# DaehwanKimLab/hisat2

Hardware: AMD Instinct MI355X
Metric: reads/sec, 101 bp PE, REDUCED-SIZE (256000000 bp, GRCh38 contig profile) linear index, --no-spliced-alignment: HI_Aligner::go per pair on the GPU (inputs and report events resident in HBM), SAM-identical to hisat2 (higher is better)
Workload: dtype u32

## Files before the change

hisat2_amd/api.py:

```python
from __future__ import annotations

import ctypes as C
import os

import numpy as np

_HERE = os.path.dirname(os.path.abspath(__file__))
DEFAULT_TAIL, DEFAULT_ALIGN_MATE = 16, 0
LIB_PATH = os.environ.get("H2G_LIBPATH") or os.path.join(_HERE, "libh2g.so")
MAX = 0xFFFFFFFF
MAX_EDITS = 32
SEED_CAP = 5

u32, u8, i32, u64, i64 = C.c_uint32, C.c_uint8, C.c_int32, C.c_uint64, C.c_int64


class LoadOpts(C.Structure):
    _fields_ = [("device", i32), ("load_local", i32)]


class IndexInfo(C.Structure):
    _fields_ = [("len", u32), ("gbwtLen", u32), ("numNodes", u32), ("lineRate", i32), ("offRate", i32),
                ("ftabChars", i32), ("eftabLen", u32), ("linear", u32), ("sideSz", u32), ("sideGbwtSz", u32),
                ("sideGbwtLen", u32), ("numSides", u32), ("offsLen", u32), ("ftabLen", u32), ("nPat", u32),
# ... 416 lines not shown
    L.h2g_rank_bench_synth.argtypes = [vp, C.c_size_t, u64, C.c_int, C.c_int, P(C.c_float), P(u64)]
    L.h2g_rank_bench_synth_sample.argtypes = [vp, C.c_size_t, C.c_size_t, vp]
    L.h2g_fm_search.argtypes = [vp, vp, C.c_size_t, u32, vp]
    L.h2g_sa_resolve.argtypes = [vp, vp, C.c_size_t, u32, vp, vp]
    L.h2g_sw_align.argtypes = [vp, vp, C.c_size_t, vp, C.c_int, P(C.c_float)]
    L.h2g_adjust_with_alt.argtypes = [vp, vp, C.c_size_t, u32, vp, vp]
    L.h2g_sa_resolve_graph.argtypes = [vp, vp, vp, C.c_size_t, u32, vp, vp]
    L.h2g_graph_lf.argtypes = [vp, vp, C.c_size_t, u32, vp, vp]
    L.h2g_fm_search_graph.argtypes = [vp, vp, C.c_size_t, u32, u32, vp, vp]
    L.h2g_index_synth_graph_sides.argtypes = [u64, u64, C.c_int, P(vp)]
    L.h2g_extend.argtypes = [vp, vp, vp, C.c_size_t, vp]
    L.h2g_seed_params_init.argtypes = [P(SeedParams), vp, C.c_int]
    L.h2g_seed_params_init.restype = None
    L.h2g_seed_extend_run.argtypes = [vp, P(SeedParams)]
    L.h2g_seed_extend_fetch.argtypes = [vp, vp, C.c_size_t, C.c_size_t]
    L.h2g_get_counters.argtypes = [vp, P(Counters)]
    L.h2g_align_params_init.argtypes = [P(AlignParams), vp]
    L.h2g_align_params_init.restype = None
    L.h2g_align_option_arity.argtypes = [C.c_char_p]
    L.h2g_align_params_apply_options.argtypes = [P(AlignParams), P(AlignPresets), P(C.c_char_p), C.c_size_t, C.c_char_p, C.c_size_t]
    L.h2g_align_params_presets.argtypes = [P(AlignParams), C.c_int, P(AlignPresets)]
    L.h2g_align_params_presets.restype = None
    L.h2g_ext_search.argtypes = [vp, vp, C.c_size_t, u32, vp, vp]
    L.h2g_local_index_of.argtypes = [vp, u32, u32]
    L.h2g_local_index_of.restype = u32
    L.h2g_set_read_names.argtypes = [vp, C.c_char_p, vp, C.c_size_t]
    L.h2g_align_run.argtypes = [vp, P(AlignParams)]
    L.h2g_align_fetch.argtypes = [vp, vp, vp, C.c_size_t, C.c_size_t]
    L.h2g_set_mates.argtypes = [vp, vp, vp, vp, C.c_char_p, vp, C.c_size_t]
    L.h2g_set_read_seeds.argtypes = [vp, vp, vp, C.c_size_t]
    L.h2g_set_read_filter.argtypes = [vp, vp, vp]
    L.h2g_set_read_ids.argtypes = [vp, vp]
    L.h2g_window_plan_create.argtypes = [u32, u32, u64, P(vp)]
    L.h2g_window_plan_add_file.argtypes = [vp, C.c_char_p, C.c_size_t]
    L.h2g_window_plan_get_info.argtypes = [vp, P(WindowPlanInfo)]
    L.h2g_window_plan_text.argtypes = [vp]
    L.h2g_window_plan_text.restype = vp
    L.h2g_window_plan_prefixes.argtypes = [vp]
    L.h2g_window_plan_prefixes.restype = vp
    L.h2g_window_plan_segments.argtypes = [vp, u64, u64, vp, C.c_size_t]
    L.h2g_window_plan_segments.restype = C.c_size_t
    L.h2g_window_plan_select.argtypes = [vp, u64, u64, P(u64), P(u64)]
    L.h2g_window_plan_select.restype = None
    L.h2g_window_plan_free.argtypes = [vp]
    L.h2g_window_plan_free.restype = None
    L.h2g_set_reads_windows.argtypes = [vp, vp, C.c_size_t, vp, C.c_size_t, u32, u32, vp, C.c_size_t]
    L.h2g_get_windows_stats.argtypes = [vp, P(WindowsStats)]
    L.h2g_fetch_reads.argtypes = [vp, P(C.c_size_t), P(C.c_size_t), P(C.c_size_t), P(C.c_int), vp, vp, vp, vp, vp]
    L.h2g_set_reads_fastq.argtypes = [vp, vp, C.c_size_t, vp, C.c_size_t, P(FastqOpts), P(FastqResult)]
    L.h2g_fetch_read_set.argtypes = [vp, C.c_int, P(C.c_size_t), P(C.c_size_t), P(C.c_size_t), vp, vp, vp, vp, vp]
    L.h2g_get_fastq_stats.argtypes = [vp, P(FastqStats)]
    L.h2g_align_pairs_run.argtypes = [vp, P(AlignParams)]
    sz = C.c_size_t
    L.h2g_sam_plan_unpaired_compact.argtypes = [vp] * 6 + [sz, vp, vp, vp, vp, sz, P(sz), vp, sz, P(sz), vp]
    L.h2g_sam_plan_paired_compact.argtypes = [vp] * 11 + [sz, vp, vp, vp, vp, vp, u32, vp, sz, P(sz), vp, sz, P(sz), vp]
    L.h2g_sam_text_unpaired.argtypes = [vp, vp, vp, sz, vp, sz, vp, sz, P(sz), vp]
    L.h2g_sam_text_paired.argtypes = [vp, vp, vp, sz, vp, sz, vp, sz, P(sz), vp]
    L.h2g_sam_text_from_plan_host.argtypes = [vp] * 11 + [sz, vp, sz, vp, sz, vp, sz, vp, sz, vp, sz, P(sz), vp]
    L.h2g_get_sam_text_stats.argtypes = [vp, P(SamTextStats)]
    L.h2g_sam_text_unpaired_planned.argtypes = [vp] * 7 + [sz, vp, vp, vp, vp, sz, P(sz), vp, sz, P(sz), vp]
    L.h2g_sam_text_paired_planned.argtypes = [vp] * 12 + [sz, vp, vp, vp, vp, vp, u32, vp, sz, P(sz), vp, sz, P(sz), vp]
    L.h2g_get_sam_plan_stats.argtypes = [vp, P(SamPlanStats), vp, sz]
    L.h2g_sam_plan_split_host.argtypes = [vp] * 11 + [sz, vp, vp, vp, vp, vp, u32, vp, sz, P(sz), vp, sz, P(sz), vp, vp]
    L.h2g_align_pairs_fetch.argtypes = [vp, vp, vp, vp, C.c_size_t, C.c_size_t]
    L.h2g_align_fetch_dense.argtypes = [vp, vp, vp, C.c_size_t, vp, C.c_size_t, C.c_size_t]
    L.h2g_align_pairs_fetch_dense.argtypes = [vp, vp, vp, C.c_size_t, vp, vp, C.c_size_t, vp, C.c_size_t, C.c_size_t]
    _lib = L
    return L


def _chk(rc, what):
    if rc != 0:
        msg = lib().h2g_last_error()
        raise H2GError(f"{what} failed: status {rc} ({msg.decode() if msg else ''})")


def mstreams_policy(units, last_bails, linear, pinned=0, light=2):
    f = lib().h2g_mstreams_policy
    f.argtypes = [C.c_ulonglong, C.c_uint, C.c_int, C.c_uint, C.c_uint]
    f.restype = C.c_uint
    return int(f(int(units), int(last_bails), int(bool(linear)), int(pinned), int(light)))


class WindowPlan:
    def __init__(self, length, step, first_rdid=0):
        self.h = C.c_void_p()
        _chk(lib().h2g_window_plan_create(length, step, first_rdid, C.byref(self.h)), "h2g_window_plan_create")
        self.len, self.step = length, step

    def add_file(self, data: bytes):
        _chk(lib().h2g_window_plan_add_file(self.h, data, len(data)), "h2g_window_plan_add_file")

    def info(self):
        i = WindowPlanInfo()
        _chk(lib().h2g_window_plan_get_info(self.h, C.byref(i)), "h2g_window_plan_get_info")
        return i

    @property
    def n_reads(self):
        return int(self.info().n_reads)

    def text(self):
        n = int(self.info().n_text)
        return np.frombuffer(C.string_at(lib().h2g_window_plan_text(self.h), n), dtype=np.uint8).copy() if n else np.zeros(0, np.uint8)

    def prefixes(self):
        n = int(self.info().n_prefix_bytes)
        return C.string_at(lib().h2g_window_plan_prefixes(self.h), n) if n else b""

    def segments(self, first=0, n=None):
        n = self.n_reads - first if n is None else n
        cnt = lib().h2g_window_plan_segments(self.h, first, n, None, 0)
        out = np.zeros(cnt, dtype=WINDOW_SEG_DTYPE)
        if cnt:
            lib().h2g_window_plan_segments(self.h, first, n, out.ctypes.data, cnt)
        return out

    def select(self, rdid_lo, rdid_hi):
        a, b = C.c_uint64(), C.c_uint64()
        lib().h2g_window_plan_select(self.h, rdid_lo, rdid_hi, C.byref(a), C.byref(b))
        return a.value, b.value

    def close(self):
        if self.h:
            lib().h2g_window_plan_free(self.h)
            self.h = C.c_void_p()


def expand_windows(text, segs, length, step, prefixes):
    text = np.asarray(text, dtype=np.uint8)
    starts, names, ids = [], [], []
    for s in segs:
        j = np.arange(int(s["n_windows"]), dtype=np.uint64)
        starts.append(np.uint64(s["text_start"]) + j * np.uint64(step))
        pre = prefixes[int(s["prefix_start"]):int(s["prefix_start"]) + int(s["prefix_len"])]
        names += [pre + str(int(s["name_off0"]) + int(k) * step).encode() for k in j]
        ids.append(((np.uint64(s["rdid0"]) + j * np.uint64(step)) & np.uint64(0xffffffff)).astype(np.uint32))
    starts = np.concatenate(starts) if starts else np.zeros(0, np.uint64)
    n = len(starts)
    codes = text[(starts[:, None] + np.arange(length, dtype=np.uint64)[None, :]).astype(np.int64)].reshape(-1)
    offs = (np.arange(n + 1, dtype=np.uint64) * np.uint64(length)).astype(np.uint32)
    noffs = np.concatenate([[0], np.cumsum([len(x) for x in names])]).astype(np.uint32)
    return codes, offs, b"".join(names), noffs, (np.concatenate(ids) if ids else np.zeros(0, np.uint32))


class Index:
    def __init__(self, base=None, device=0, synth_sides=None, seed=20260925, graph=False):
        L = lib()
        self.h = C.c_void_p()
        if synth_sides is not None and graph:
            _chk(L.h2g_index_synth_graph_sides(int(synth_sides), int(seed), int(device), C.byref(self.h)),
                 "h2g_index_synth_graph_sides")
        elif synth_sides is not None:
            _chk(L.h2g_index_synth_sides(int(synth_sides), int(seed), int(device), C.byref(self.h)), "h2g_index_synth_sides")
        else:
            o = LoadOpts(device, 1)
            _chk(L.h2g_index_load(base.encode(), C.byref(o), C.byref(self.h)), "h2g_index_load")
        self.info = IndexInfo()
        _chk(L.h2g_index_get_info(self.h, C.byref(self.info)), "h2g_index_get_info")

    def dense_sa(self, verify=False):
        st, nd = u32(0), u64(0)
        _chk(lib().h2g_index_dense_sa_check(self.h, C.byref(st), C.byref(nd) if verify else None), "h2g_index_dense_sa_check")
        return bool(st.value), (int(nd.value) if verify else None)

    def dense_lsa(self, verify=False):
# ... 452 lines not shown
```

hisat2_amd/csrc/h2g_go_args.h:

```cpp
#pragma once
#include <hip/hip_runtime.h>
#include <atomic>
#include "h2g_align.h"
#include "h2g_graph.h"
#include "h2g_fast.h"

enum : unsigned {
	H2G_CNT_RANK = 0, H2G_CNT_SIDE = 1, H2G_CNT_STEPS = 2, H2G_CNT_EXT = 3,
	H2G_CNT_ALIGNED = 4, H2G_CNT_OVERFLOW = 5,
	H2G_CNT_FAST_DONE = 6, H2G_CNT_FAST_BAILED = 7,
	H2G_CNT_BENCH_SUM = 6, H2G_CNT_BENCH_CHECKSUM = 7,
	H2G_CNT_WORK_FAST = 12, H2G_CNT_WORK_DRAIN = 13, H2G_CNT_WORK_MAIN = 14, H2G_CNT_WORK_SECOND = 15,
	H2G_CNT_PROF_GO = 16, H2G_CNT_PROF_GO_CTL = 80,
	H2G_CNT_NO_SECOND = 64,
	H2G_CNT_FAST_BAIL_WHY = 96,
	H2G_CNT_FAST_RANK = 120, H2G_CNT_FAST_SIDE = 121, H2G_CNT_FAST_STEPS = 122, H2G_CNT_FAST_ALIGNED = 123,
	H2G_CNT_DRAIN_OFF = 120,
	H2G_CNT_OVF_CURSOR = 124, H2G_CNT_LEDITS_CURSOR = 126,
	H2G_CNT_PROF_FAST = 128, H2G_CNT_PROF_FAST_SITE = 176, H2G_CNT_PROF_FAST_TRIPS = 208,
	H2G_CNT_SECOND = 256,
	H2G_CNT_PROF_FAST_BINS = 512,
#ifdef H2G_GO_PROF
	H2G_CNT_BLOCK = 1024
#else
// ... 70 lines not shown
			uint16_t v;
			while((v = __atomic_load_n(&ring[q][pos], __ATOMIC_RELAXED)) == EMPTY) __builtin_amdgcn_s_sleep(1);
			__atomic_store_n(&ring[q][pos], EMPTY, __ATOMIC_RELAXED);
			*slot = v;
		}
		return n;
	}
};

template <auto K, class... Args>
static int launch_large_lds(unsigned grid, unsigned threads, unsigned lds, hipStream_t st, const Args&... args) {
	static std::atomic<unsigned long long> lds_ok{0};
	int dev = 0; (void)hipGetDevice(&dev);
	const unsigned long long bit = 1ull << (dev & 63);
	if(!(lds_ok.load(std::memory_order_relaxed) & bit)) { if(hipFuncSetAttribute((const void*)K, hipFuncAttributeMaxDynamicSharedMemorySize, 160 * 1024) != hipSuccess) (void)hipGetLastError(); lds_ok.fetch_or(bit, std::memory_order_relaxed); }
	hipLaunchKernelGGL(K, dim3(grid), dim3(threads), lds, st, args...);
	return (int)hipGetLastError();
}

struct GoArgs {
	h2g::DGfm g; h2g::DRef ref; h2g::DLocalSet ls; h2g::DAlts alts; h2g::DSpliceDB ssdb;
	h2g::DReads rd1, rd2;
	h2g::AlnParams P;
	const char* names1; const uint32_t* noffs1;
	const char* names2; const uint32_t* noffs2;
	uint8_t* pool; size_t ws_stride;
	size_t slot_off, gsl_off;
	uint8_t* gws_base; size_t gws_stride;
	uint8_t* sw_base; size_t sw_stride;
	uint8_t* sc_base;
	h2g::MachOut O;
	unsigned long long* counters;
	uint32_t* work;
	const uint32_t* list;
	const uint32_t* nlist;
	uint32_t paired;
	uint32_t dbg_read; uint32_t* dbg_buf;
	uint32_t rdid_base;
	uint32_t defer_overflow;
};
#define H2G_PK_LANE_WORDS_HOST (H2G_PK_WORDS + H2G_PK_WORDS / 2)

struct GoUnitDesc {
	size_t ws_bytes, slot_off, gsl_off;
	size_t gws_bytes;
	int waves;
	uint32_t threads, slots;
	uint32_t lds_ring_bytes, lds_pack_bytes;
	uint32_t caps[5];
	size_t (*sw_bytes)(uint32_t maxlen, int wide);
	int (*launch)(const GoArgs*, const h2g::DExonTbl*, const h2g::XlPairs*, unsigned grid, hipStream_t);
};
#define H2G_GO_DECLARE(NAME) extern "C" const GoUnitDesc* h2g_go_unit_##NAME();
H2G_GO_DECLARE(linear) H2G_GO_DECLARE(graph) H2G_GO_DECLARE(linear_big) H2G_GO_DECLARE(graph_big)
H2G_GO_DECLARE(linear_spl) H2G_GO_DECLARE(linear_spl_big) H2G_GO_DECLARE(graph_spl) H2G_GO_DECLARE(graph_spl_big)
H2G_GO_DECLARE(linear_xl) H2G_GO_DECLARE(graph_xl) H2G_GO_DECLARE(linear_spl_xl) H2G_GO_DECLARE(graph_spl_xl)

struct FastArgs {
	h2g::DGfm g; h2g::DRef ref; h2g::DLocalSet ls;
	h2g::DReads rd1, rd2;
	h2g::AlnParams P;
	const char* names1; const uint32_t* noffs1;
	const char* names2; const uint32_t* noffs2;
	uint32_t* slots;
	h2g::FastOut O;
	unsigned long long* counters;
	uint32_t* work;
	uint32_t* bail_list; uint32_t* bail_count;
	uint32_t total, paired;
	h2g::DAlts alts;
	uint8_t* gws_base; size_t gws_stride;
	uint8_t* sc_base;
	uint32_t tail;
	uint32_t dbg_read; uint32_t* dbg_buf;
	uint32_t orphan_T; uint32_t* orphan_list; uint32_t* orphan_count;
	const uint32_t* adopt_list; const uint32_t* adopt_count; const uint32_t* adopt_slots;
	uint32_t cnt_off;
	uint32_t adopt_slot_words;
	uint32_t mate_handover;
	h2g::DSpliceDB ssdb;
	uint32_t rdid_base;
	uint32_t* ps0;
};
extern "C" int h2g_ps0_launch(const FastArgs* a, uint32_t units, bool paired, hipStream_t st);
struct FastUnitDesc {
	int (*launch)(const FastArgs* a, unsigned grid, hipStream_t);
	int (*launch_drain)(const FastArgs* a, unsigned grid, hipStream_t);
	uint32_t threads, lds_bytes;
	uint32_t slots, slot_bytes;
	uint32_t gws_bytes;
};
extern "C" const FastUnitDesc* h2g_go_fast_unit();
extern "C" const FastUnitDesc* h2g_go_fast_am_unit();
extern "C" const FastUnitDesc* h2g_go_fast_graph_unit();
extern "C" const FastUnitDesc* h2g_go_fast_spl_unit();
```

hisat2_amd/csrc/h2g_k_ps0.hip:

```cpp
#include "h2g_go_args.h"

using namespace h2g;

#define PS0_THREADS 256

__global__ __launch_bounds__(PS0_THREADS, 6) void k_ps0(const FastArgs* __restrict__ A, uint32_t units)
{
	__shared__ uint32_t s_pk[H2G_PK_WORDS * PS0_THREADS];
	const bool paired = A->paired != 0;
	const uint32_t sh = paired ? 2u : 1u;
	const uint32_t t = blockIdx.x * PS0_THREADS + threadIdx.x;
	const uint32_t unit = t >> sh, x = t & ((1u << sh) - 1u), mate = x >> 1;
	const uint32_t lane = threadIdx.x & 63u;
	const bool live = unit < units;
	const DReads& rd = mate ? A->rd2 : A->rd1;
	uint32_t* const pk = s_pk + (threadIdx.x & ~1u);
	bool ok = true;
	uint32_t rl = 0;
	if(live) {
		rl = rd.offs[unit + 1] - rd.offs[unit];
		if((x & 1u) == 0) {
			ok = fg_pack_read(rd, unit, pk, PS0_THREADS);
			if(rd.qc && !rd.qc[unit]) ok = false;
		}
	}
	__syncthreads();
	const unsigned long long bad = __ballot(!ok);
	const bool absent = ((bad >> (lane & ~((1u << sh) - 1u))) & ((1ull << (1u << sh)) - 1ull)) != 0;
	if(!live) return;
	uint32_t rec[FG_PS0_WORDS] = {FG_PS0_ABSENT, FG_PS0_ABSENT, FG_PS0_ABSENT, FG_PS0_ABSENT};
	if(!absent) {
		SeqView sv;
		sv.fwc = nullptr; sv.q = nullptr; sv.len = rl; sv.fw = (x & 1u) == 0;
		sv.pk = pk; sv.pk_stride = PS0_THREADS; sv.pk_nomask = true;
		h2g_fm_hit fh;
		partial_search_item(A->g, sv, 0, A->P.pseudogeneStop != 0, A->P.anchorStop != 0, A->P.khits, &fh);
		fg_ps0_pack(fh, rec);
	}
	*reinterpret_cast<uint4*>(A->ps0 + ((size_t)unit * 4 + x) * FG_PS0_WORDS) = make_uint4(rec[0], rec[1], rec[2], rec[3]);
}

extern "C" int h2g_ps0_launch(const FastArgs* a, uint32_t units, bool paired, hipStream_t st) {
	if(units == 0) return 0;
	const unsigned long long lanes = (unsigned long long)units * (paired ? 4u : 2u);
	hipLaunchKernelGGL(k_ps0, dim3((unsigned)((lanes + PS0_THREADS - 1) / PS0_THREADS)), dim3(PS0_THREADS), 0, st, a, units);
	return (int)hipGetLastError();
}
```

hisat2_amd/csrc/h2g_kernels.hip:

```cpp
#include <hip/hip_runtime.h>
#include <stdio.h>
#include <stdlib.h>
#include <string>
#include <vector>
#include <thread>
#include <atomic>
#include <memory>
#include <chrono>
#include <algorithm>
#define H2G_EXT_OPTS 0
#define H2G_HAPLOTYPE 0
#include "h2g_core.h"
#include "h2g_dev.h"
#include "h2g_parts.h"
#include "h2g_host_index.h"
#include "h2g_align.h"
#include "h2g_graph.h"
#include "h2g_sw.h"
#include "h2g_graph_staged.h"
#include "h2g_local_pack.h"
#include "h2g_splice_host.h"
#include "h2g_splice_db_host.h"
#include "h2g_windows.h"
#include "h2g_fastq.h"
// ... 2 lines not shown
#include <chrono>
#include "h2g_go_args.h"

using namespace h2g;

static thread_local char g_err[512] = "";
static int set_err(const char* what, hipError_t e) {
	snprintf(g_err, sizeof g_err, "%s: %s", what, hipGetErrorString(e));
	return H2G_ERR_DEVICE;
}
#define HIPCHK(call) do { hipError_t e_ = (call); if(e_ != hipSuccess) return set_err(#call, e_); } while(0)

extern "C" const char* h2g_last_error(void) { return g_err; }

struct h2g_index {
	DevStream dense_st;
	HostIndex host;
	bool synthetic = false;
	int device = 0;
	DGfm dg;
	DRef dr;
	DLocalSet dls;
	DAlts dalts;
	bool has_local = false;
	uint32_t n_local = 0;
	bool has_splice_alts = false;
	std::vector<h2g_splice_site> alt_sites;
	DSpliceDB dssdb;
	DExonTbl dexons;
	DevBuf<uint8_t> d_ssdb[4];
	HostSpliceDB h_ssdb;
	const float* d_spl[3] = {nullptr, nullptr, nullptr};
	std::vector<DLocalDesc> h_ldesc;
	std::vector<DevBuf<uint8_t>> allocs;
	uint64_t device_bytes = 0;
	uint32_t* d_sa_dense = nullptr; uint8_t* d_sa_dist = nullptr;
	DevEvent dense_ev;
	std::atomic<bool> dense_ready{false};
	double dense_ms = 0.0;
	bool dense_synced = false;
	uint32_t* d_lsa = nullptr; uint64_t* d_lsa_base = nullptr;
	uint64_t lsa_rows = 0;
	DevEvent lsa_ev;
	std::atomic<bool> lsa_ready{false};
	double lsa_ms = 0.0;
	~h2g_index() { if(dense_st) { (void)hipSetDevice(device); (void)hipStreamSynchronize(dense_st); } }
};
struct IndexFree { void operator()(h2g_index* ix) const { h2g_index_free(ix); } };
typedef std::unique_ptr<h2g_index, IndexFree> IndexPtr;
static DGfm dg_now(h2g_index* ix) {
	DGfm g = ix->dg;
	if(!ix->d_sa_dist) return g;
	if(!ix->dense_ready.load(std::memory_order_acquire)) {
		if(hipEventQuery(ix->dense_ev) != hipSuccess) { (void)hipGetLastError(); return g; }
		ix->dense_ready.store(true, std::memory_order_release);
	}
	g.sa_dense = ix->d_sa_dense; g.sa_dist = ix->d_sa_dist;
	return g;
}

static DLocalSet dls_now(h2g_index* ix) {
	DLocalSet l = ix->dls;
	if(!ix->d_lsa) return l;
	if(!ix->lsa_ready.load(std::memory_order_acquire)) {
		if(hipEventQuery(ix->lsa_ev) != hipSuccess) { (void)hipGetLastError(); return l; }
		ix->lsa_ready.store(true, std::memory_order_release);
	}
	l.lsa = ix->d_lsa; l.lsa_base = ix->d_lsa_base;
	return l;
}

#define H2G_MSTREAMS_MAX 8
#define H2G_MSTREAMS_LIGHT_DEFAULT 2
#define H2G_NBUF (H2G_MSTREAMS_MAX + 1)
#define H2G_FAST_RESERVE_DEFAULT 0
#define H2G_DEFAULT_TAIL 16
#define H2G_ORPHAN_T 512
#define H2G_ORPHAN_MIN_UNITS 200000
#define H2G_DRAIN_GRID 64
#define H2G_FAST_POOLS 3
#ifndef H2G_DEFAULT_PS0
#define H2G_DEFAULT_PS0 1
#endif
#define H2G_DEFAULT_ALIGN_MATE 0
#define H2G_DEFAULT_FAST_SPLICED 0
#define H2G_MACH_MAXGRID 48u
#define H2G_MACH_TOTAL 128u
#define H2G_MAX_BATCHES 16
struct BatchCtx {
	size_t n_reads = 0; uint32_t max_read_len = 0;
	DevBuf<uint8_t> d_codes; DevBuf<uint32_t> d_offs; DevBuf<char> d_quals; bool has_quals = false;
	DevBuf<char> d_names; DevBuf<uint32_t> d_name_offs; bool has_names = false;
	DevBuf<uint8_t> d_codes2; DevBuf<uint32_t> d_offs2; DevBuf<char> d_quals2, d_names2; DevBuf<uint32_t> d_name_offs2; bool has_mates = false, has_quals2 = false;
	DevBuf<ReadOut> d_rout; DevBuf<h2g_alnres> d_aln; uint32_t aln_slots = 0;
	DevBuf<PairOut> d_pout; DevBuf<h2g_alnres> d_paln[2]; uint32_t pair_slots = 0;
	DevBuf<uint32_t> d_seeds; bool has_seeds = false, has_seeds2 = false;
	DevBuf<uint8_t> d_qc; bool has_qc = false;
	DevBuf<uint32_t> d_ids; bool has_ids = false;
	hipError_t ensure_reads(size_t max_reads, size_t max_bases) {
		hipError_t e = d_codes.ensure(max_bases + 64);
		if(e == hipSuccess) e = d_quals.ensure(max_bases + 64);
		return e != hipSuccess ? e : d_offs.ensure(max_reads + 1);
	}
	hipError_t reserve_names(size_t nb, size_t max_reads) {
		if(d_names.size() >= nb + 64 && d_name_offs) return hipSuccess;
		const hipError_t e = d_names.reset(nb + 64);
		return e != hipSuccess ? e : d_name_offs.reset(max_reads + 1);
	}
	hipError_t ensure_mates(size_t max_reads, size_t max_bases, size_t nb2) {
		hipError_t e = d_codes2.ensure(max_bases + 64);
		if(e == hipSuccess) e = d_quals2.ensure(max_bases + 64);
		if(e == hipSuccess) e = d_offs2.ensure(max_reads + 1);
		if(e == hipSuccess) e = d_name_offs2.ensure(max_reads + 1);
		return e != hipSuccess ? e : d_names2.reset(nb2 + 64);
	}
};
enum Tm {
	TM_PRIM0, TM_PRIM1,
	TM_SEED0, TM_SEED_MID, TM_SEED1,
	TM_RUN0, TM_MAIN1, TM_MAIN0, TM_RUN1,
	TM_EXT1,
	TM_FAST1,
	TM_SET0, TM_SET1,
	TM_N
};
struct h2g_stream {
	h2g_index* ix = nullptr;
	DevStream st;
	DevStream mst[H2G_MSTREAMS_MAX];
	DevStream dst;
	unsigned n_mst = 0;
	unsigned mstreams = 0;
	unsigned mstreams_light = H2G_MSTREAMS_LIGHT_DEFAULT;
	unsigned rot = 0;
	bool st2_busy = false;
	unsigned gen = 0;
	struct RunSet {
		DevEvent ev_fast, ev_mach;
		DevEvent ev_bails;
		DevEvent ev_drain;
		DevBuf<uint32_t> bail_list;
		DevBuf<uint32_t> orphans;
		DevBuf<FastArgs> fast_args, drain_args;
	} run[H2G_NBUF];
	DevBuf<unsigned long long> d_counters;
	PinnedBuf<uint32_t> h_bails;
	PinnedBuf<FastArgs> h_fast_args;
	unsigned long long* counters(const RunSet& b) const { return d_counters + (&b - run) * H2G_CNT_BLOCK; }
	uint32_t& h_bail(const RunSet& b) const { return h_bails[&b - run]; }
	FastArgs* h_fast(const RunSet& b) const { return h_fast_args + 2 * (&b - run); }
	FastArgs* h_drain(const RunSet& b) const { return h_fast_args + 2 * (&b - run) + 1; }
	unsigned long long* cnt_cur = nullptr;
	uint32_t last_bails = 0;
	size_t max_reads = 0, max_bases = 0;
	BatchCtx batch[H2G_MAX_BATCHES];
	unsigned cur_batch = 0;
	BatchCtx& cur() { return batch[cur_batch]; }
	const BatchCtx& cur() const { return batch[cur_batch]; }
	DevBuf<h2g_seed_result> d_seed;
	struct GoPool {
		DevBuf<uint8_t> ws;
		DevBuf<uint8_t> gws;
		DevBuf<uint8_t> sw; size_t sw_stride = 0, sw_lanes = 0;
		DevBuf<uint8_t> sc;
	};
	struct MachStream {
		DevEvent ev_rot;
		GoPool main, second;
		DevBuf<uint32_t> ovf_list;
		bool warmed = false;
	} mach[H2G_MSTREAMS_MAX];
	hipStream_t stream_of(const MachStream& m) const { return mst[&m - mach]; }
	const MachStream* ovf_cur = mach;
	DevBuf<uint32_t> dbg_buf;
	struct FastPool {
		DevBuf<uint8_t> slots;
		DevBuf<uint32_t> ps0;
		DevEvent ev_last;
	} fpool[H2G_FAST_POOLS];
	size_t orphan_cap = 0;
	DevBuf<uint8_t> d_drain_slots;
	DevBuf<uint8_t> d_drain_sc;
	bool dst_busy = false;
	DevEvent ev_dr[2];
	bool ran_drain = false;
	const uint32_t* orph_cur = nullptr;
	DevBuf<uint8_t> d_fast_gws;
	DevBuf<uint8_t> d_fast_sc;
	bool ran_fast = false;
	struct Tune { int fast, blocks_per_cu, pair_slots, no_second_pass; unsigned mach_div, mach_min, mach_total; int mach_total_auto = 1; int fast_reserve; long dbg_read;
	              int tail, tail_auto = 1, align_mate, orphan, drain_grid, mate_handover, ps0, fast_spliced; } tune = {};
	h2g_align_params last_p; int last_paired = -1;
	DevBuf<uint8_t> d_sw_ws;
	DevBuf<SwLaneState> d_sw_states;
	PartArea<h2g_edit> ledits; DevBuf<uint32_t> d_ledits_cur;
	unsigned ledits_touched = 0;
	PartArea<h2g_alnres> paln_ovf;
	DevBuf<uint32_t> d_xlp_at; PartArea<uint32_t> xlp; DevBuf<uint32_t> d_xlp_cur;
	const PairOut* xlp_pout = nullptr;
	DevBuf<uint8_t> d_tmp[4];
	uint64_t tmp_gen = 0;
	struct CompactFetch { bool valid = false, paired = false; uint64_t gen = 0; unsigned batch = 0; size_t first = 0, n = 0; const uint8_t* d_rec[2] = {nullptr, nullptr}; uint64_t bytes[2] = {0, 0};
	                      const uint64_t* d_boffs[2] = {nullptr, nullptr};  } cfetch;
	DevBuf<uint8_t> d_sam[5];
	uint64_t samtab_uid = 0, samtab_gen = 0; uint32_t samtab_nrefs = 0, samtab_names = 0, samtab_rg = 0, samtab_nalts = 0; int32_t samtab_strand = 0;
	DevEvent ev_sam[4];
	h2g_sam_text_stats sam_stats = {};
	DevBuf<uint8_t> d_plan[5];
	DevEvent ev_plan[4];
	h2g_sam_plan_stats plan_stats = {};
	std::vector<uint8_t> plan_classes;
	DevEvent tm[TM_N];
	bool ran_seed = false, ran_align = false;
	h2g_counters last;
	h2g_windows_stats win_stats = {};
	h2g_fastq_stats fq_stats = {};
	DevBuf<unsigned long long> d_warm_cnt;
	DevBuf<uint8_t> d_warm_rows;
	~h2g_stream() {
		if(st) (void)hipStreamSynchronize(st);
		if(dst) (void)hipStreamSynchronize(dst);
		for(unsigned k = 0; k < n_mst; k++) (void)hipStreamSynchronize(mst[k]);
	}
};
struct StreamFree { void operator()(h2g_stream* s) const { h2g_stream_free(s); } };

struct Stager {
	enum { T = 6, NB = 2 };
	static constexpr size_t CH = (size_t)16 << 20;
	DevStream st[T]; PinnedBuf<uint8_t> buf[T][NB]; DevEvent ev[T][NB];
	int device = 0; bool ok = false;
	bool init(int dev) {
		device = dev; ok = true;
		for(int t = 0; t < T && ok; t++) {
			ok = st[t].create(hipStreamNonBlocking) == hipSuccess;
			for(int b = 0; b < NB && ok; b++) ok = buf[t][b].ensure(CH) == hipSuccess && ev[t][b].create(hipEventDisableTiming) == hipSuccess;
		}
		if(!ok) (void)hipGetLastError();
		return ok;
	}
	bool copy(void* dst, const void* src, size_t bytes) {
		return gather(dst, bytes, [src](uint8_t* out, size_t off, size_t len) { memcpy(out, (const uint8_t*)src + off, len); });
	}
	template <class F>
	bool gather(void* dst, size_t bytes, F fill) {
		std::atomic<bool> good{true};
		std::thread th[T];
		const size_t nch = (bytes + CH - 1) / CH;
		for(int t = 0; t < T; t++) th[t] = std::thread([&, t]() {
			if(hipSetDevice(device) != hipSuccess) { good = false; return; }
			size_t n = 0;
			for(size_t k = (size_t)t; k < nch; k += T, n++) {
				const int b = (int)(n % NB);
				const size_t off = k * CH, len = bytes - off < CH ? bytes - off : CH;
				if(n >= NB && hipEventSynchronize(ev[t][b]) != hipSuccess) { good = false; return; }
				fill(buf[t][b], off, len);
				if(hipMemcpyAsync((uint8_t*)dst + off, buf[t][b], len, hipMemcpyHostToDevice, st[t]) != hipSuccess || hipEventRecord(ev[t][b], st[t]) != hipSuccess) { good = false; return; }
			}
			if(hipStreamSynchronize(st[t]) != hipSuccess) good = false;
		});
		for(int t = 0; t < T; t++) th[t].join();
		if(!good) (void)hipGetLastError();
		return good;
	}
};
static int index_alloc(h2g_index* ix, size_t bytes, uint8_t** out) {
	DevBuf<uint8_t> b;
	HIPCHK(b.reset(bytes));
	*out = b;
	ix->allocs.push_back(std::move(b));
	ix->device_bytes += bytes;
	return H2G_OK;
}
static int upload_raw(h2g_index* ix, const void* src, size_t n, const void** out, size_t pad, Stager* sg) {
	uint8_t* p = nullptr;
	int rc;
	if((rc = index_alloc(ix, n + pad, &p))) return rc;
	HIPCHK(hipMemset(p + n, 0, pad));
	if(n) {
		if(sg && sg->ok && n >= ((size_t)32 << 20)) { if(!sg->copy(p, src, n)) { snprintf(g_err, sizeof g_err, "index upload through the staging buffers failed"); return H2G_ERR_DEVICE; } }
		else HIPCHK(hipMemcpy(p, src, n, hipMemcpyHostToDevice));
	}
	*out = p;
	return H2G_OK;
}
template <typename T>
static int upload(h2g_index* ix, const std::vector<T>& v, const T** out, size_t pad = 64, Stager* sg = nullptr) {
	const void* p = nullptr;
	const int rc = upload_raw(ix, v.data(), v.size() * sizeof(T), &p, pad ? pad : 64, sg);
	*out = (const T*)p;
	return rc;
}

extern "C" void h2g_load_opts_init(h2g_load_opts* o) { o->device = 0; o->load_local = 1; }

#define H2G_DENSE_CHUNK 4096u
__global__ __launch_bounds__(256) void k_sa_dense_build(DGfm g, uint32_t* sa_dense, uint8_t* sa_dist) {
	const uint64_t wave = (blockIdx.x * (uint64_t)blockDim.x + threadIdx.x) / 64u;
	const uint64_t base = wave * H2G_DENSE_CHUNK;
	if(base >= g.gbwtLen) return;
	const uint64_t lim = base + H2G_DENSE_CHUNK < g.gbwtLen ? base + H2G_DENSE_CHUNK : g.gbwtLen;
	sa_dense_build_rows(g, base + (threadIdx.x & 63u), 64u, lim, sa_dense, sa_dist);
}
__global__ __launch_bounds__(256) void k_sa_dense_check(DGfm g, const uint32_t* sa_dense, const uint8_t* sa_dist, unsigned long long* ndiff) {
	const uint64_t stride = (uint64_t)gridDim.x * blockDim.x;
// ... 406 lines not shown
__global__ void k_synth_write(uint8_t* sides, const uint32_t* cnt, uint64_t nsides, const uint32_t* chunk, uint32_t sideSz) {
	uint64_t t = blockIdx.x * (uint64_t)blockDim.x + threadIdx.x;
	if(t >= SYNTH_CHUNKS) return;
	uint64_t per = (nsides + SYNTH_CHUNKS - 1) / SYNTH_CHUNKS, a = t * per, b = a + per < nsides ? a + per : nsides;
	uint32_t run[4];
	for(int k = 0; k < 4; k++) run[k] = chunk[t * 4 + k];
	for(uint64_t s = a; s < b; s++) {
		uint32_t* occ = reinterpret_cast<uint32_t*>(sides + s * sideSz + sideSz - 16);
		for(int k = 0; k < 4; k++) { occ[k] = run[k]; run[k] += cnt[s * 4 + k]; }
	}
}

static h2g_status synth_sides(uint64_t num_sides, uint64_t seed, int device, uint32_t sideSz, h2g_index** out) {
	const uint32_t syms = sideSz == 64 ? 192u : H2G_GSIDE_SYMS;
	if(!out || num_sides == 0 || num_sides * (uint64_t)syms >= 0xffffffffull) return H2G_ERR_ARG;
	int ndev = 0;
	if(hipGetDeviceCount(&ndev) != hipSuccess || ndev <= 0) { snprintf(g_err, sizeof g_err, "no HIP device"); return H2G_ERR_DEVICE; }
	HIPCHK(hipSetDevice(device));
	IndexPtr ixp(new h2g_index());
	h2g_index* const ix = ixp.get();
	ix->synthetic = true;
	ix->device = device;
	DevBuf<uint8_t> sbuf;
	DevBuf<uint32_t> cnt, tot, chunk;
	const size_t bytes = num_sides * sideSz + 256;
	{
		const char* mt = getenv("H2G_SIDES_MTYPE");
		const bool unc = mt && !strcmp(mt, "uncached");
		if(unc || (mt && !strcmp(mt, "finegrained"))) {
			void* p = nullptr;
			HIPCHK(hipExtMallocWithFlags(&p, bytes, unc ? hipDeviceMallocUncached : hipDeviceMallocFinegrained));
			sbuf = DevBuf<uint8_t>((uint8_t*)p, bytes);
		}
		else HIPCHK(sbuf.reset(bytes));
	}
	uint8_t* const sides = sbuf;
	HIPCHK(cnt.reset(num_sides * 4));
	HIPCHK(tot.reset(4));
	ix->allocs.push_back(std::move(sbuf));
	ix->device_bytes = num_sides * sideSz;
	hipLaunchKernelGGL(k_synth_fill, dim3((unsigned)((num_sides + 255) / 256)), dim3(256), 0, 0, sides, cnt.get(), num_sides, seed, sideSz);
	HIPCHK(chunk.reset(SYNTH_CHUNKS * 4));
	hipLaunchKernelGGL(k_synth_chunk_sum, dim3(SYNTH_CHUNKS / 256), dim3(256), 0, 0, (const uint32_t*)cnt, num_sides, chunk.get());
	hipLaunchKernelGGL(k_synth_chunk_scan, dim3(1), dim3(64), 0, 0, chunk.get(), tot.get());
	hipLaunchKernelGGL(k_synth_write, dim3(SYNTH_CHUNKS / 256), dim3(256), 0, 0, sides, (const uint32_t*)cnt, num_sides, (const uint32_t*)chunk, sideSz);
	uint32_t totals[4];
	HIPCHK(hipMemcpy(totals, tot, 16, hipMemcpyDeviceToHost));
	GfmParams& p = ix->host.g.p;
	uint32_t len = (uint32_t)(num_sides * syms - 1);
	if(sideSz == 64) p.init(len, len + 1, len + 1, 6, 4, 10, 0, 4);
	else p.init(len - 1000, len + 1, len - 500, 7, 4, 10, 0, 4);
	p.numSides = (uint32_t)num_sides;
	ix->host.g.fchr[0] = 0;
	for(int c = 0; c < 4; c++) ix->host.g.fchr[c + 1] = ix->host.g.fchr[c] + totals[c];
	fill_dgfm(ix->host.g, 16, &ix->dg);
	ix->dg.sides = sides;
	ix->dg.nZ = 0;
	*out = ixp.release();
	return H2G_OK;
}
extern "C" h2g_status h2g_index_synth_sides(uint64_t num_sides, uint64_t seed, int device, h2g_index** out) {
	return synth_sides(num_sides, seed, device, 64, out);
}
extern "C" h2g_status h2g_index_synth_graph_sides(uint64_t num_sides, uint64_t seed, int device, h2g_index** out) {
	return synth_sides(num_sides, seed, device, 128, out);
}

struct Knob { const char *key, *env; long def; void (*set)(h2g_stream::Tune&, long); int h2g_stream::Tune::* is_auto; };
#define H2G_KNOB(key, env, def, member, is_auto) {key, env, def, [](h2g_stream::Tune& t, long v) { t.member = (decltype(t.member))v; }, is_auto}
static const Knob g_knobs[] = {
	H2G_KNOB("fast",           "H2G_GO_FAST",            1,                        fast,           nullptr),
	H2G_KNOB("blocks_per_cu",  "H2G_GO_BLOCKS_PER_CU",   0,                        blocks_per_cu,  nullptr),
	H2G_KNOB("pair_slots",     "H2G_PAIR_SLOTS",         0,                        pair_slots,     nullptr),
	H2G_KNOB("no_second_pass", "H2G_GO_NO_SECOND_PASS",  0,                        no_second_pass, nullptr),
	H2G_KNOB("mach_div",       "H2G_MACH_DIV",           0,                        mach_div,       nullptr),
	H2G_KNOB("mach_min",       "H2G_MACH_MIN",           4,                        mach_min,       nullptr),
	H2G_KNOB("dbg_read",       "H2G_GO_DBG_READ",        -1,                       dbg_read,       nullptr),
	H2G_KNOB("tail",           "H2G_FAST_TAIL",          H2G_DEFAULT_TAIL,         tail,           &h2g_stream::Tune::tail_auto),
	H2G_KNOB("align_mate",     "H2G_FAST_AM",            H2G_DEFAULT_ALIGN_MATE,   align_mate,     nullptr),
	H2G_KNOB("orphan",         "H2G_FAST_ORPHAN",        -1,                       orphan,         nullptr),
	H2G_KNOB("drain_grid",     "H2G_DRAIN_GRID",         H2G_DRAIN_GRID,           drain_grid,     nullptr),
	H2G_KNOB("mate_handover",  "H2G_FAST_MATE_HANDOVER", -1,                       mate_handover,  nullptr),
	H2G_KNOB("ps0",            "H2G_FAST_PS0",           -1,                       ps0,            nullptr),
	H2G_KNOB("fast_spliced",   "H2G_FAST_SPLICED",       H2G_DEFAULT_FAST_SPLICED, fast_spliced,   nullptr),
	H2G_KNOB("mach_total",     "H2G_MACH_TOTAL",         H2G_MACH_TOTAL,           mach_total,     &h2g_stream::Tune::mach_total_auto),
	H2G_KNOB("fast_reserve",   "H2G_FAST_RESERVE",       H2G_FAST_RESERVE_DEFAULT, fast_reserve,   nullptr),
};
#undef H2G_KNOB
static unsigned clamp_mstreams(long m) { return (unsigned)(m < 1 ? 1 : m > H2G_MSTREAMS_MAX ? H2G_MSTREAMS_MAX : m); }


extern "C" h2g_status h2g_stream_create(h2g_index* ix, size_t max_reads, size_t max_bases, h2g_stream** out) {
	if(!ix || !out) return H2G_ERR_ARG;
	HIPCHK(hipSetDevice(ix->device));
	std::unique_ptr<h2g_stream, StreamFree> sp(new h2g_stream());
	h2g_stream* const s = sp.get();
	s->ix = ix; s->max_reads = max_reads; s->max_bases = max_bases;
	HIPCHK(s->st.create(hipStreamNonBlocking));
	for(int k = 0; k < H2G_MSTREAMS_MAX; k++) { HIPCHK(s->mst[k].create(hipStreamNonBlocking)); HIPCHK(s->mach[k].ev_rot.create(hipEventDisableTiming)); }
	HIPCHK(s->dst.create(hipStreamNonBlocking));
	HIPCHK(s->h_fast_args.ensure(2 * H2G_NBUF));
	HIPCHK(s->h_bails.ensure(H2G_NBUF)); for(int k = 0; k < H2G_NBUF; k++) s->h_bails[k] = 0;
	for(h2g_stream::RunSet& b : s->run) { HIPCHK(b.ev_fast.create(hipEventDisableTiming)); HIPCHK(b.ev_mach.create(hipEventDisableTiming)); HIPCHK(b.ev_bails.create(hipEventDisableTiming)); HIPCHK(b.ev_drain.create(hipEventDisableTiming)); }
	for(h2g_stream::FastPool& fp : s->fpool) HIPCHK(fp.ev_last.create(hipEventDisableTiming));
	for(int k = 0; k < 2; k++) HIPCHK(s->ev_dr[k].create());
	for(DevEvent& e : s->tm) HIPCHK(e.create());
	HIPCHK(s->d_counters.ensure(H2G_NBUF * H2G_CNT_BLOCK));
	HIPCHK(hipMemset(s->d_counters, 0, s->d_counters.bytes()));
	s->cnt_cur = s->d_counters;
	if(max_reads) {
		HIPCHK(s->batch[0].ensure_reads(max_reads, max_bases));
		HIPCHK(s->d_seed.ensure(max_reads * 2));
		HIPCHK(hipMemset(s->d_seed, 0, s->d_seed.bytes()));
	}
	memset(&s->last, 0, sizeof s->last);
	for(const Knob& k : g_knobs) {
		const char* const e = getenv(k.env);
		k.set(s->tune, e ? atol(e) : k.def);
		if(e && k.is_auto) s->tune.*k.is_auto = 0;
	}
	if(const char* const e = getenv("H2G_MSTREAMS")) s->mstreams = clamp_mstreams(atol(e));
	if(const char* const e = getenv("H2G_MSTREAMS_LIGHT")) s->mstreams_light = clamp_mstreams(atol(e));
	*out = sp.release();
	return H2G_OK;
}

extern "C" void h2g_stream_free(h2g_stream* s) { delete s; }

static hipError_t sync_mach(h2g_stream* s) {
	if(!s->st2_busy) return hipSuccess;
	for(unsigned k = 0; k < s->n_mst; k++) { const hipError_t e = hipStreamSynchronize(s->mst[k]); if(e != hipSuccess) return e; }
	s->st2_busy = false;
	return hipSuccess;
}
static hipError_t sync_all(h2g_stream* s) {
	hipError_t e = hipStreamSynchronize(s->st);
	if(e == hipSuccess && s->dst_busy) { e = hipStreamSynchronize(s->dst); s->dst_busy = false; }
	if(e == hipSuccess && s->st2_busy) { e = sync_mach(s); s->st2_busy = false; }
	return e;
}
extern "C" void* h2g_stream_hip(h2g_stream* s) { return s ? (void*)s->st : nullptr; }
extern "C" h2g_status h2g_stream_sync(h2g_stream* s) {
	if(!s) return H2G_ERR_ARG;
	HIPCHK(sync_all(s));
	return H2G_OK;
}

extern "C" h2g_status h2g_stream_select_batch(h2g_stream* s, unsigned k) {
	if(!s || k >= H2G_MAX_BATCHES) return H2G_ERR_ARG;
	if(k == s->cur_batch) return H2G_OK;
	HIPCHK(hipSetDevice(s->ix->device));
	const BatchCtx& out = s->cur();
	BatchCtx& in = s->batch[k];
	if(s->max_reads) HIPCHK(in.ensure_reads(s->max_reads, s->max_bases));
	if(!in.d_paln[1] && out.d_pout && out.d_paln[1]) {
		HIPCHK(in.d_pout.ensure(s->max_reads));
		for(int m = 0; m < 2; m++) HIPCHK(in.d_paln[m].reserve(out.d_paln[m].size()));
		in.pair_slots = out.pair_slots;
		HIPCHK(hipMemsetAsync(in.d_pout, 0, in.d_pout.bytes(), s->st));
		for(int m = 0; m < 2; m++) HIPCHK(hipMemsetAsync(in.d_paln[m], 0, in.d_paln[m].bytes(), s->st));
	}
	if(!in.d_aln && out.d_rout && out.d_aln) {
		HIPCHK(in.d_rout.ensure(s->max_reads));
		HIPCHK(in.d_aln.reserve(out.d_aln.size()));
		in.aln_slots = out.aln_slots;
		HIPCHK(hipMemsetAsync(in.d_rout, 0, in.d_rout.bytes(), s->st));
		HIPCHK(hipMemsetAsync(in.d_aln, 0, in.d_aln.bytes(), s->st));
	}
	s->cur_batch = k;
	s->tmp_gen++;
	return H2G_OK;
}

static int tmp_buf(h2g_stream* s, int slot, size_t bytes, void** out) {
	s->tmp_gen++;
	const hipError_t e = s->d_tmp[slot].reserve(bytes + 256);
	*out = s->d_tmp[slot];
	return e == hipSuccess ? H2G_OK : set_err("tmp_buf", e);
}

extern "C" h2g_status h2g_set_reads(h2g_stream* s, const uint8_t* codes, const uint32_t* offs, const char* quals, size_t n) {
	if(s) HIPCHK(sync_all(s));
	if(!s || !codes || !offs || n > s->max_reads) return H2G_ERR_ARG;
	s->tmp_gen++;
	BatchCtx& B = s->cur();
	size_t nb = offs[n];
	if(nb > s->max_bases) return H2G_ERR_ARG;
	uint32_t mx = 0;
	for(size_t i = 0; i < n; i++) { const uint32_t l = offs[i + 1] - offs[i]; if(l > mx) mx = l; }
	B.max_read_len = mx;
	HIPCHK(hipMemcpyAsync(B.d_codes, codes, nb, hipMemcpyHostToDevice, s->st));
	HIPCHK(hipMemcpyAsync(B.d_offs, offs, (n + 1) * 4, hipMemcpyHostToDevice, s->st));
	B.has_quals = quals != nullptr;
	if(quals) HIPCHK(hipMemcpyAsync(B.d_quals, quals, nb, hipMemcpyHostToDevice, s->st));
	HIPCHK(sync_all(s));
	B.n_reads = n;
	B.has_names = false;
	B.has_mates = false;
	B.has_seeds = B.has_seeds2 = false;
	B.has_qc = false;
	B.has_ids = false;
	s->ledits_touched = 0;
	return H2G_OK;
}

static DReads dreads(const h2g_stream* s) {
	DReads r;
	r.codes = s->cur().d_codes; r.offs = s->cur().d_offs; r.quals = s->cur().has_quals ? s->cur().d_quals : nullptr; r.n = (uint32_t)s->cur().n_reads;
	return r;
}

static unsigned grid_for(size_t n, unsigned block) {
	size_t g = (n + block - 1) / block;
	const size_t cap = 256 * 16;
	return (unsigned)(g < 1 ? 1 : (g > cap ? cap : g));
}

__device__ __forceinline__ uint32_t synth_row(uint64_t h, uint32_t n) { return (uint32_t)(((h >> 32) * (uint64_t)n) >> 32); }
__global__ __launch_bounds__(256) void k_rank_v0(DGfm g, const uint32_t* rows, const uint8_t* cs, uint32_t* out,
                                                 size_t n, uint64_t seed, int synth)
{
	size_t stride = (size_t)gridDim.x * blockDim.x;
	for(size_t i = blockIdx.x * (size_t)blockDim.x + threadIdx.x; i < n; i += stride) {
		uint32_t row; int c;
		if(synth) { uint64_t h = splitmix64(seed + i); row = synth_row(h, g.gbwtLen); c = (int)((h >> 40) & 3); }
		else { row = rows[i]; c = cs[i]; }
		out[i] = rank64(g, row, c);
	}
}

__global__ __launch_bounds__(512) void k_rank_v0_512(DGfm g, const uint32_t* rows, const uint8_t* cs, uint32_t* out, size_t n, uint64_t seed, int synth)
{
	size_t stride = (size_t)gridDim.x * blockDim.x;
	for(size_t i = blockIdx.x * (size_t)blockDim.x + threadIdx.x; i < n; i += stride) {
		uint32_t row; int c;
		if(synth) { uint64_t h = splitmix64(seed + i); row = synth_row(h, g.gbwtLen); c = (int)((h >> 40) & 3); }
		else { row = rows[i]; c = cs[i]; }
		out[i] = rank64(g, row, c);
	}
}

__global__ __launch_bounds__(256) void k_rank_v0_sampled(DGfm g, uint32_t* out, size_t n, uint64_t seed, unsigned long long* sum)
{
	size_t stride = (size_t)gridDim.x * blockDim.x;
	unsigned long long acc = 0;
	for(size_t i = blockIdx.x * (size_t)blockDim.x + threadIdx.x; i < n; i += stride) {
		const uint64_t h = splitmix64(seed + i);
		const uint32_t r = rank64(g, synth_row(h, g.gbwtLen), (int)((h >> 40) & 3));
		if((i & 255) == 0) out[i] = r;
		acc += (unsigned long long)r * (unsigned long long)((i & 1023) + 1);
	}
	for(int o = 32; o > 0; o >>= 1) acc += __shfl_xor(acc, o);
	if((threadIdx.x & 63) == 0) atomicAdd(sum, acc);
}

template <int UNROLL>
__global__ __launch_bounds__(256) void k_rank_v1(DGfm g, const uint32_t* rows, const uint8_t* cs, uint32_t* out,
                                                 size_t n, uint64_t seed, int synth)
{
	const unsigned lane = threadIdx.x & 63, sub = lane & 3;
	const size_t ngroups = ((size_t)gridDim.x * blockDim.x) >> 2;
	const size_t gid = (blockIdx.x * (size_t)blockDim.x + threadIdx.x) >> 2;
	for(size_t base = gid * UNROLL; base < n; base += ngroups * UNROLL) {
		uint32_t row[UNROLL], sideNum[UNROLL], charOff[UNROLL]; int c[UNROLL]; uint4 v[UNROLL];
#pragma unroll
		for(int u = 0; u < UNROLL; u++) {
			size_t i = base + u;
			bool ok = i < n;
			if(synth) { uint64_t h = splitmix64(seed + (ok ? i : 0)); row[u] = synth_row(h, g.gbwtLen); c[u] = (int)((h >> 40) & 3); }
			else { row[u] = ok ? rows[i] : 0; c[u] = ok ? cs[i] : 0; }
			sideNum[u] = row[u] / 192u; charOff[u] = row[u] - sideNum[u] * 192u;
			v[u] = reinterpret_cast<const uint4*>(g.sides + (size_t)sideNum[u] * 64)[sub];
		}
#pragma unroll
		for(int u = 0; u < UNROLL; u++) {
			uint64_t w0 = v[u].x | ((uint64_t)v[u].y << 32), w1 = v[u].z | ((uint64_t)v[u].w << 32);
			int n0 = (int)charOff[u] - 64 * (int)sub;
// ... 953 lines not shown
	h2g_ghit scratch;
	for(size_t i = blockIdx.x * (size_t)blockDim.x + threadIdx.x; i < n; i += stride) {
		SeqView sv = seq_view(rd, (uint32_t)(i >> 1), (i & 1) == 0);
		resolve_extend_item(g, ref, sc, sv, &out[i], &scratch);
		nsteps += out[i].nsteps; next += out[i].ncoords;
	}
	wave_add(counters + H2G_CNT_STEPS, nsteps);
	wave_add(counters + H2G_CNT_EXT, next);
}

extern "C" void h2g_seed_params_init(h2g_seed_params* p, const h2g_index* ix, int no_spliced) {
	p->pseudogeneStop = (ix && ix->dg.linear && !no_spliced) ? 1 : 0;
	p->anchorStop = 1;
	p->khits = (ix && !ix->dg.linear) ? 10 : 5;
	p->search_variant = 0;
}

extern "C" h2g_status h2g_seed_extend_run(h2g_stream* s, const h2g_seed_params* p) {
	if(!s || !p) return H2G_ERR_ARG;
	int rc;
	if((rc = need_reads(s)) || (rc = need_linear(s))) return rc;
	HIPCHK(hipSetDevice(s->ix->device));
	const size_t n = s->cur().n_reads * 2;
	HIPCHK(hipMemsetAsync(s->d_counters, 0, 4 * sizeof(unsigned long long), s->st));
	DScoring sc;
	HIPCHK(hipEventRecord(s->tm[TM_SEED0], s->st));
	hipLaunchKernelGGL(k_seed_search, dim3(grid_for(n, 256)), dim3(256), 0, s->st, s->ix->dg, dreads(s), *p, s->d_seed, s->d_counters);
	HIPCHK(hipEventRecord(s->tm[TM_SEED_MID], s->st));
	hipLaunchKernelGGL(k_seed_resolve_extend, dim3(grid_for(n, 256)), dim3(256), 0, s->st, dg_now(s->ix), s->ix->dr, dreads(s), sc, s->d_seed, s->d_counters);
	HIPCHK(hipEventRecord(s->tm[TM_SEED1], s->st));
	HIPCHK(hipGetLastError());
	s->ran_seed = true;
	return H2G_OK;
}

extern "C" h2g_status h2g_seed_extend_fetch(h2g_stream* s, h2g_seed_result* out, size_t first_read, size_t n_reads) {
	if(!s || !out || first_read + n_reads > s->cur().n_reads) return H2G_ERR_ARG;
	HIPCHK(hipMemcpyAsync(out, s->d_seed + first_read * 2, n_reads * 2 * sizeof *out, hipMemcpyDeviceToHost, s->st));
	HIPCHK(sync_all(s));
	return H2G_OK;
}

static_assert(sizeof(h2g_alnres) == sizeof(AlnRec), "h2g_alnres must mirror AlnRec");
static_assert(sizeof(h2g_read_result) == 40, "h2g_read_result layout");
static_assert(sizeof(h2g_pair_result) == sizeof(PairOut), "h2g_pair_result must mirror PairOut");
static_assert(H2G_PAIR_CAP == AL_MAX_PAIRS, "pair capacity");

extern "C" int h2g_device_count(void) { int n = 0; if(hipGetDeviceCount(&n) != hipSuccess) { (void)hipGetLastError(); return 0; } return n; }

extern "C" void h2g_align_params_init(h2g_align_params* p, const h2g_index* ix) { align_params_defaults(p, !ix || ix->dg.linear); }

extern "C" h2g_status h2g_set_read_names(h2g_stream* s, const char* bytes, const uint32_t* offs, size_t n) {
	if(s) HIPCHK(sync_all(s));
	if(!s || !bytes || !offs || n != s->cur().n_reads || n == 0) return H2G_ERR_ARG;
	s->tmp_gen++;
	HIPCHK(hipSetDevice(s->ix->device));
	BatchCtx& B = s->cur();
	size_t nb = offs[n];
	HIPCHK(B.reserve_names(nb, s->max_reads));
	HIPCHK(hipMemcpyAsync(B.d_names, bytes, nb, hipMemcpyHostToDevice, s->st));
	HIPCHK(hipMemcpyAsync(B.d_name_offs, offs, (n + 1) * 4, hipMemcpyHostToDevice, s->st));
	HIPCHK(sync_all(s));
	B.has_names = true;
	return H2G_OK;
}

extern "C" h2g_status h2g_set_mates(h2g_stream* s, const uint8_t* codes2, const uint32_t* offs2, const char* quals2,
                                    const char* nb2, const uint32_t* noffs2, size_t n)
{
	if(s) HIPCHK(sync_all(s));
	if(!s || !codes2 || !offs2 || !nb2 || !noffs2 || n != s->cur().n_reads || n == 0) return H2G_ERR_ARG;
	if(offs2[n] > s->max_bases) return H2G_ERR_ARG;
	s->tmp_gen++;
	BatchCtx& B = s->cur();
	for(size_t i = 0; i < n; i++) { const uint32_t l = offs2[i + 1] - offs2[i]; if(l > B.max_read_len) B.max_read_len = l; }
	HIPCHK(hipSetDevice(s->ix->device));
	HIPCHK(B.ensure_mates(s->max_reads, s->max_bases, noffs2[n]));
	HIPCHK(hipMemcpyAsync(B.d_codes2, codes2, offs2[n], hipMemcpyHostToDevice, s->st));
	HIPCHK(hipMemcpyAsync(B.d_offs2, offs2, (n + 1) * 4, hipMemcpyHostToDevice, s->st));
	B.has_quals2 = quals2 != nullptr;
	if(quals2) HIPCHK(hipMemcpyAsync(B.d_quals2, quals2, offs2[n], hipMemcpyHostToDevice, s->st));
	HIPCHK(hipMemcpyAsync(B.d_names2, nb2, noffs2[n], hipMemcpyHostToDevice, s->st));
	HIPCHK(hipMemcpyAsync(B.d_name_offs2, noffs2, (n + 1) * 4, hipMemcpyHostToDevice, s->st));
	HIPCHK(sync_all(s));
	B.has_mates = true;
	return H2G_OK;
}

extern "C" h2g_status h2g_set_read_seeds(h2g_stream* s, const uint32_t* seeds1, const uint32_t* seeds2, size_t n) {
	if(s) HIPCHK(sync_all(s));
	if(!s) return H2G_ERR_ARG;
	BatchCtx& B = s->cur();
	if(!seeds1) { B.has_seeds = B.has_seeds2 = false; return H2G_OK; }
	if(n != B.n_reads || n == 0) return H2G_ERR_ARG;
	HIPCHK(hipSetDevice(s->ix->device));
	HIPCHK(B.d_seeds.ensure(2 * s->max_reads));
	HIPCHK(hipMemcpyAsync(B.d_seeds, seeds1, n * sizeof(uint32_t), hipMemcpyHostToDevice, s->st));
	if(seeds2) HIPCHK(hipMemcpyAsync(B.d_seeds + s->max_reads, seeds2, n * sizeof(uint32_t), hipMemcpyHostToDevice, s->st));
	HIPCHK(sync_all(s));
	B.has_seeds = true; B.has_seeds2 = seeds2 != nullptr;
	return H2G_OK;
}

extern "C" h2g_status h2g_set_read_ids(h2g_stream* s, const uint32_t* ids) {
	if(s) HIPCHK(sync_all(s));
	if(!s) return H2G_ERR_ARG;
	BatchCtx& B = s->cur();
	if(!ids) { B.has_ids = false; return H2G_OK; }
	const size_t n = B.n_reads;
	if(n == 0 || n > s->max_reads) return H2G_ERR_ARG;
	HIPCHK(hipSetDevice(s->ix->device));
	HIPCHK(B.d_ids.ensure(s->max_reads));
	HIPCHK(hipMemcpyAsync(B.d_ids, ids, n * sizeof(uint32_t), hipMemcpyHostToDevice, s->st));
	HIPCHK(sync_all(s));
	B.has_ids = true;
	return H2G_OK;
}

__global__ __launch_bounds__(256) void k_win_codes(const uint8_t* __restrict__ text, const h2g_win::DSeg* __restrict__ segs, uint32_t n_segs, uint32_t len, uint32_t step,
                                                   uint64_t n_bytes, uint8_t* __restrict__ codes)
{
	const uint64_t chunks = (n_bytes + 15) / 16;
	for(uint64_t c = (uint64_t)blockIdx.x * blockDim.x + threadIdx.x; c < chunks; c += (uint64_t)gridDim.x * blockDim.x) {
		const uint64_t b0 = c * 16;
		const uint32_t m = n_bytes - b0 < 16 ? (uint32_t)(n_bytes - b0) : 16u;
		h2g_win::CodeCursor cur;
		cur.seek(segs, n_segs, len, step, b0);
		uint32_t w[4] = {0, 0, 0, 0};
		for(uint32_t k = 0; k < m; k++) w[k >> 2] |= (uint32_t)text[cur.next()] << (8 * (k & 3));
		*(uint4*)(codes + b0) = make_uint4(w[0], w[1], w[2], w[3]);
	}
}
__global__ __launch_bounds__(256) void k_win_meta(const h2g_win::DSeg* __restrict__ segs, uint32_t n_segs, uint32_t len, uint32_t step, uint32_t n, const char* __restrict__ prefixes,
                                                  uint32_t* __restrict__ offs, uint32_t* __restrict__ ids, uint32_t* __restrict__ name_offs, char* __restrict__ names)
{
	for(uint32_t r = blockIdx.x * blockDim.x + threadIdx.x; r <= n; r += gridDim.x * blockDim.x) {
		offs[r] = r * len;
		if(r == n) { name_offs[r] = segs[n_segs].name_first; break; }
		const h2g_win::DSeg s = segs[h2g_win::seg_of(segs, n_segs, r)];
		const uint32_t j = r - s.first_read;
		ids[r] = s.rdid0 + j * step;
		const uint32_t at = h2g_win::name_start(s, step, j);
		name_offs[r] = at;
		h2g_win::write_name(s, step, j, prefixes, names + at);
	}
}

extern "C" h2g_status h2g_set_reads_windows(h2g_stream* s, const uint8_t* text, size_t n_text, const h2g_window_seg* segs, size_t n_segs, uint32_t len, uint32_t step,
                                            const char* prefixes, size_t n_prefix_bytes)
{
	if(s) HIPCHK(sync_all(s));
	if(!s || !text || !segs || n_segs == 0 || n_segs >= 0xffffffffull || len == 0 || (!prefixes && n_prefix_bytes)) return H2G_ERR_ARG;
	s->tmp_gen++;
	BatchCtx& B = s->cur();
	std::vector<h2g_win::DSeg> ds(n_segs + 1);
	uint64_t n = 0, nb = 0, lo = UINT64_MAX, hi = 0;
	for(size_t k = 0; k < n_segs; k++) {
		const h2g_window_seg& x = segs[k];
		const uint64_t last = x.text_start + (uint64_t)(x.n_windows ? x.n_windows - 1 : 0) * step;
		if(x.n_windows == 0 || last + len > n_text || last < x.text_start || (uint64_t)x.prefix_start + x.prefix_len > n_prefix_bytes) {
			snprintf(g_err, sizeof g_err, "h2g_set_reads_windows: segment %zu names text or prefix bytes that were not given", k); return H2G_ERR_ARG;
		}
		if(x.text_start < lo) lo = x.text_start;
		if(last + len > hi) hi = last + len;
		h2g_win::DSeg& d = ds[k];
		d.name_off0 = x.name_off0; d.rdid0 = (uint32_t)x.rdid0; d.first_read = (uint32_t)n; d.name_first = (uint32_t)nb;
		d.prefix_start = x.prefix_start; d.prefix_len = x.prefix_len;
		n += x.n_windows;
		nb += (uint64_t)x.n_windows * x.prefix_len + h2g_win::width_sum(x.name_off0, step, x.n_windows);
		if(n > s->max_reads || n * len > s->max_bases || n * len > 0xffffffffull || nb > 0xffffffffull) {
			snprintf(g_err, sizeof g_err, "h2g_set_reads_windows: the windows exceed the stream's %zu reads / %zu bases, or their names 4 GB", s->max_reads, s->max_bases); return H2G_ERR_ARG;
		}
	}
	if(hi - lo > 0xffffffffull) { snprintf(g_err, sizeof g_err, "h2g_set_reads_windows: the segments span more than 4 G bases of text"); return H2G_ERR_ARG; }
	for(size_t k = 0; k < n_segs; k++) ds[k].text_start = (uint32_t)(segs[k].text_start - lo);
	memset(&ds[n_segs], 0, sizeof ds[n_segs]);
	ds[n_segs].first_read = (uint32_t)n; ds[n_segs].name_first = (uint32_t)nb;
	HIPCHK(hipSetDevice(s->ix->device));
	HIPCHK(B.reserve_names(nb, s->max_reads));
	HIPCHK(B.d_ids.ensure(s->max_reads));
	void *d_text, *d_segs, *d_pre;
	int rc;
	if((rc = tmp_buf(s, 0, hi - lo, &d_text)) || (rc = tmp_buf(s, 1, ds.size() * sizeof(h2g_win::DSeg), &d_segs)) || (rc = tmp_buf(s, 2, n_prefix_bytes, &d_pre))) return (h2g_status)rc;
	HIPCHK(hipMemcpyAsync(d_text, text + lo, hi - lo, hipMemcpyHostToDevice, s->st));
	HIPCHK(hipMemcpyAsync(d_segs, ds.data(), ds.size() * sizeof(h2g_win::DSeg), hipMemcpyHostToDevice, s->st));
	if(n_prefix_bytes) HIPCHK(hipMemcpyAsync(d_pre, prefixes, n_prefix_bytes, hipMemcpyHostToDevice, s->st));
	const uint64_t n_bytes = n * len;
	HIPCHK(hipEventRecord(s->tm[TM_SET0], s->st));
	k_win_codes<<<grid_for((n_bytes + 15) / 16, 256), 256, 0, s->st>>>((const uint8_t*)d_text, (const h2g_win::DSeg*)d_segs, (uint32_t)n_segs, len, step, n_bytes, B.d_codes);
	k_win_meta<<<grid_for(n + 1, 256), 256, 0, s->st>>>((const h2g_win::DSeg*)d_segs, (uint32_t)n_segs, len, step, (uint32_t)n, (const char*)d_pre, B.d_offs, B.d_ids, B.d_name_offs, B.d_names);
	HIPCHK(hipGetLastError());
	HIPCHK(hipEventRecord(s->tm[TM_SET1], s->st));
	HIPCHK(sync_all(s));
	s->win_stats.bytes_uploaded = (hi - lo) + ds.size() * sizeof(h2g_win::DSeg) + n_prefix_bytes;
	s->win_stats.bytes_written = n_bytes + (n + 1) * 8 + n * 4 + nb;
	HIPCHK(hipEventElapsedTime(&s->win_stats.kernel_ms, s->tm[TM_SET0], s->tm[TM_SET1]));
	B.n_reads = n;
	B.max_read_len = len;
	B.has_quals = false;
	B.has_names = true;
	B.has_mates = false;
	B.has_seeds = B.has_seeds2 = false;
	B.has_qc = false;
	B.has_ids = true;
	s->ledits_touched = 0;
	return H2G_OK;
}
extern "C" h2g_status h2g_get_windows_stats(h2g_stream* s, h2g_windows_stats* out) {
	if(!s || !out) return H2G_ERR_ARG;
	*out = s->win_stats;
	return H2G_OK;
}

extern "C" h2g_status h2g_fetch_reads(h2g_stream* s, size_t* n_reads, size_t* n_bases, size_t* n_name_bytes, int* has_ids, uint8_t* codes, uint32_t* offs, char* names,
                                      uint32_t* name_offs, uint32_t* ids)
{
	if(!s) return H2G_ERR_ARG;
	HIPCHK(sync_all(s));
	const BatchCtx& B = s->cur();
	const size_t n = B.n_reads;
	uint32_t nb = 0, nn = 0;
	HIPCHK(hipSetDevice(s->ix->device));
	if(n) HIPCHK(hipMemcpy(&nb, B.d_offs + n, 4, hipMemcpyDeviceToHost));
	if(n && B.has_names) HIPCHK(hipMemcpy(&nn, B.d_name_offs + n, 4, hipMemcpyDeviceToHost));
	if(n_reads) *n_reads = n;
	if(n_bases) *n_bases = nb;
	if(n_name_bytes) *n_name_bytes = nn;
	if(has_ids) *has_ids = B.has_ids ? 1 : 0;
	if(n == 0) return H2G_OK;
	if((ids && !B.has_ids) || ((names || name_offs) && !B.has_names)) return H2G_ERR_ARG;
	if(codes && nb) HIPCHK(hipMemcpy(codes, B.d_codes, nb, hipMemcpyDeviceToHost));
	if(offs) HIPCHK(hipMemcpy(offs, B.d_offs, (n + 1) * 4, hipMemcpyDeviceToHost));
	if(names && nn) HIPCHK(hipMemcpy(names, B.d_names, nn, hipMemcpyDeviceToHost));
	if(name_offs) HIPCHK(hipMemcpy(name_offs, B.d_name_offs, (n + 1) * 4, hipMemcpyDeviceToHost));
	if(ids) HIPCHK(hipMemcpy(ids, B.d_ids, n * 4, hipMemcpyDeviceToHost));
	return H2G_OK;
}

extern "C" h2g_status h2g_set_read_filter(h2g_stream* s, const uint8_t* pass1, const uint8_t* pass2) {
	if(s) HIPCHK(sync_all(s));
	if(!s) return H2G_ERR_ARG;
	BatchCtx& B = s->cur();
	if(!pass1 && !pass2) { B.has_qc = false; return H2G_OK; }
	const size_t n = B.n_reads;
	if(n == 0 || n > s->max_reads) return H2G_ERR_ARG;
	HIPCHK(hipSetDevice(s->ix->device));
	HIPCHK(B.d_qc.ensure(2 * s->max_reads));
	if(pass1) HIPCHK(hipMemcpyAsync(B.d_qc, pass1, n, hipMemcpyHostToDevice, s->st)); else HIPCHK(hipMemsetAsync(B.d_qc, 1, n, s->st));
	if(pass2) HIPCHK(hipMemcpyAsync(B.d_qc + s->max_reads, pass2, n, hipMemcpyHostToDevice, s->st)); else HIPCHK(hipMemsetAsync(B.d_qc + s->max_reads, 1, n, s->st));
	HIPCHK(sync_all(s));
	B.has_qc = true;
	return H2G_OK;
}

extern "C" h2g_status h2g_combine_with(h2g_stream* s, const h2g_align_params* p, h2g_ghit* a, const h2g_ghit* b, const int64_t* minsc, size_t n, uint32_t* ok) {
	if(!s || !a || !b || !minsc || !ok || n == 0) return H2G_ERR_ARG;
	int rc;
	if((rc = need_reads(s))) return rc;
	if(s->ix->synthetic) { snprintf(g_err, sizeof g_err, "synthetic index: rank only"); return H2G_ERR_ARG; }
	const bool linear = s->ix->dg.linear != 0;
	for(size_t i = 0; i < n; i++) {
		if(a[i].read >= s->cur().n_reads || b[i].read != a[i].read || a[i].tidx >= s->ix->dr.nrefs || b[i].tidx >= s->ix->dr.nrefs || a[i].nedits > H2G_MAX_EDITS || b[i].nedits > H2G_MAX_EDITS) return H2G_ERR_ARG;
	}
	if(s->cur().max_read_len > H2G_COMBINE_MAXLEN) return H2G_ERR_ARG;
	h2g_align_params hp;
	if(p) hp = *p; else align_params_defaults(&hp, linear);
	AlnParams P = aln_params_from(hp, hp.no_spliced_alignment != 0, linear);
	if(!hp.no_spliced_alignment) { P.sc.donor_sum = s->ix->d_spl[0]; P.sc.acc_sum1 = s->ix->d_spl[1]; P.sc.acc_sum2 = s->ix->d_spl[2]; }
	HIPCHK(hipSetDevice(s->ix->device));
	unsigned grid = grid_for(n, 256);
	if(grid > 64) grid = 64;
	void *da, *db, *dm, *dscr;
	const size_t ab = n * sizeof(h2g_ghit);
	if((rc = tmp_buf(s, 0, 2 * ab, &da)) || (rc = tmp_buf(s, 1, n * 8, &dm)) || (rc = tmp_buf(s, 2, n * 4, &db)) ||
	   (rc = tmp_buf(s, 3, (size_t)grid * 256 * 2 * H2G_COMBINE_MAXLEN * sizeof(int64_t), &dscr))) return rc;
	h2g_ghit* const d_a = (h2g_ghit*)da; h2g_ghit* const d_b = d_a + n;
	HIPCHK(hipMemcpyAsync(d_a, a, ab, hipMemcpyHostToDevice, s->st));
	HIPCHK(hipMemcpyAsync(d_b, b, ab, hipMemcpyHostToDevice, s->st));
	HIPCHK(hipMemcpyAsync(dm, minsc, n * 8, hipMemcpyHostToDevice, s->st));
	hipLaunchKernelGGL(k_combine, dim3(grid), dim3(256), 0, s->st, s->ix->dr, s->ix->dalts, dreads(s), P, d_a, (const h2g_ghit*)d_b, (const int64_t*)dm, n, (uint32_t*)db, (int64_t*)dscr);
	HIPCHK(hipGetLastError());
	HIPCHK(hipMemcpyAsync(a, d_a, ab, hipMemcpyDeviceToHost, s->st));
	HIPCHK(hipMemcpyAsync(ok, db, n * 4, hipMemcpyDeviceToHost, s->st));
	HIPCHK(sync_all(s));
	return H2G_OK;
}

static int need_alignable(h2g_stream* s) {
	if(s->ix->synthetic) { snprintf(g_err, sizeof g_err, "synthetic index: rank only"); return H2G_ERR_ARG; }
	const DGfm& g = s->ix->dg;
	if(g.linear && g.lineRate == 6) return H2G_OK;
	if(!g.linear && g.lineRate == 7) return H2G_OK;
	snprintf(g_err, sizeof g_err, "unsupported side geometry (lineRate %u)", g.lineRate);
	return H2G_ERR_UNSUPPORTED;
}

static const GoUnitDesc& go_unit(bool linear, bool big, bool spliced = false, bool xl = false) {
	static const GoUnitDesc* (*const u[2][2][3])() = {
		{{h2g_go_unit_graph, h2g_go_unit_graph_big, h2g_go_unit_graph_xl}, {h2g_go_unit_linear, h2g_go_unit_linear_big, h2g_go_unit_linear_xl}},
		{{h2g_go_unit_graph_spl, h2g_go_unit_graph_spl_big, h2g_go_unit_graph_spl_xl}, {h2g_go_unit_linear_spl, h2g_go_unit_linear_spl_big, h2g_go_unit_linear_spl_xl}}};
	return *u[spliced ? 1 : 0][linear ? 1 : 0][xl ? 2 : big ? 1 : 0]();
}
static const FastUnitDesc& fast_unit(bool linear, bool spliced, bool align_mate) {
	return *(!linear ? h2g_go_fast_graph_unit : spliced ? h2g_go_fast_spl_unit : align_mate ? h2g_go_fast_am_unit : h2g_go_fast_unit)();
}

static int go_pool_for(h2g_stream* s, h2g_stream::GoPool& pl, const GoUnitDesc& u, size_t slots, size_t lanes, uint32_t bowtie2_dp, GoArgs* a) {
	const size_t wsb = u.ws_bytes, gwb = u.gws_bytes;
	HIPCHK(pl.ws.reserve(slots * wsb));
	a->pool = pl.ws; a->ws_stride = wsb; a->slot_off = u.slot_off; a->gsl_off = u.gsl_off;
	a->gws_base = nullptr; a->gws_stride = gwb;
	if(gwb) {
		HIPCHK(pl.gws.reserve(lanes * gwb));
		a->gws_base = pl.gws;
	}
	HIPCHK(pl.sc.reserve(lanes * (size_t)(2 * H2G_COMBINE_MAXLEN * sizeof(int64_t))));
	a->sc_base = pl.sc;
	a->sw_base = nullptr; a->sw_stride = 0;
	if(bowtie2_dp) {
		const uint32_t swlen = s->cur().max_read_len > H2G_SW_MAX_ROWS ? (uint32_t)H2G_SW_MAX_ROWS : s->cur().max_read_len;
		bool wide = false;
		for(uint32_t l = 1; l <= swlen && !wide; l++) wide = sw_wide_for(min_score_for(a->P, l));
		const size_t stride = (u.sw_bytes(swlen, wide ? 1 : 0) + 255) & ~(size_t)255;
		if(pl.sw_stride < stride || pl.sw_lanes < lanes) {
			pl.sw_stride = 0; pl.sw_lanes = 0;
			HIPCHK(pl.sw.reset(stride * lanes));
			HIPCHK(hipMemset(pl.sw, 0, stride * lanes));
			pl.sw_stride = stride; pl.sw_lanes = lanes;
		}
		a->sw_base = pl.sw; a->sw_stride = pl.sw_stride;
	}
	return H2G_OK;
}


static int go_check(h2g_stream* s, const h2g_align_params* p, bool paired) {
	int rc;
	if((rc = need_reads(s)) || (rc = need_alignable(s))) return rc;
	if(!s->ix->has_local) { snprintf(g_err, sizeof g_err, "align: index loaded without local (.5/.6) indexes"); return H2G_ERR_ARG; }
	if(!s->cur().has_names || (paired && !s->cur().has_mates)) { snprintf(g_err, sizeof g_err, "align: read names (h2g_set_read_names)%s not set", paired ? " / mates (h2g_set_mates)" : ""); return H2G_ERR_ARG; }
	if(paired && s->cur().has_seeds && !s->cur().has_seeds2) { snprintf(g_err, sizeof g_err, "align: explicit seeds without mate 2's (h2g_set_read_seeds seeds2)"); return H2G_ERR_ARG; }
	if(p->n_ceil_type < 1 || p->n_ceil_type > 4) { snprintf(g_err, sizeof g_err, "align: n_ceil_type %u (1 C, 2 L, 3 S, 4 G)", p->n_ceil_type); return H2G_ERR_ARG; }
	if(p->sc_min < 1) { snprintf(g_err, sizeof g_err, "align: sc_min %d (--sp): the soft-clipping penalty must be at least 1", p->sc_min); return H2G_ERR_ARG; }
	if(p->mm_max < 1) { snprintf(g_err, sizeof g_err, "align: mm_max %d (--mp): the maximum mismatch penalty must be at least 1", p->mm_max); return H2G_ERR_ARG; }
	if(p->mm_max < p->mm_min) { snprintf(g_err, sizeof g_err, "align: mm_max %d is less than mm_min %d (--mp)", p->mm_max, p->mm_min); return H2G_ERR_ARG; }
	if(p->rdg_linear < 1 || p->rfg_linear < 1) { snprintf(g_err, sizeof g_err, "align: rdg_linear %d / rfg_linear %d (--rdg, --rfg): a gap extension penalty must be at least 1", p->rdg_linear, p->rfg_linear); return H2G_ERR_ARG; }
	if(!p->no_spliced_alignment) {
		if(p->pen_canintronlen_type < 1 || p->pen_canintronlen_type > 4 || p->pen_noncanintronlen_type < 1 || p->pen_noncanintronlen_type > 4 ||
		   p->min_intronlen < 20 || p->max_intronlen < p->min_intronlen || p->pen_cansplice < 0 || p->pen_noncansplice < 0 ||
		   p->min_anchor_len < 1 || p->min_anchor_len_noncan < 1) {
			snprintf(g_err, sizeof g_err, "align: splice scoring outside its range (intron-length function type 1..4, 20 <= min_intronlen <= max_intronlen, penalties >= 0)");
			return H2G_ERR_ARG;
		}
		if(p->max_intronlen > H2G_SPL_MAXLEN) {
			snprintf(g_err, sizeof g_err, "align: --max-intronlen %u is beyond the %u bases a splice edit holds", p->max_intronlen, (unsigned)H2G_SPL_MAXLEN);
			return H2G_ERR_UNSUPPORTED;
		}
	}
	if(p->khits == 0 || p->khits > H2G_KHITS_MAX || p->kseeds < p->khits || p->kseeds > H2G_KSEEDS_MAX) {
		snprintf(g_err, sizeof g_err, "align: -k %u / --max-seeds %u outside the built range (1 <= -k <= %u, -k <= --max-seeds <= %u)", p->khits, p->kseeds, (unsigned)H2G_KHITS_MAX, (unsigned)H2G_KSEEDS_MAX);
		return H2G_ERR_ARG;
	}
	if(p->bowtie2_dp > 2 || p->pe_orientation > 2 || p->min_frag_len >= (1u << 24)) return H2G_ERR_ARG;
	if(p->pen_conflictsplice < 0) { snprintf(g_err, sizeof g_err, "align: --pen-conflictsplice arg must be at least 0"); return H2G_ERR_ARG; }
	if(p->max_alts_tried && p->max_alts_tried < 8) { snprintf(g_err, sizeof g_err, "align: --max-altstried arg must be at least 8"); return H2G_ERR_ARG; }
	if(p->bowtie2_dp && s->cur().max_read_len == 0) return H2G_ERR_ARG;
	return H2G_OK;
}

struct GoPlan {
	bool linear, spl, xl, big_main, fast, second;
	bool fast_spl;
	const GoUnitDesc *U, *L;
	unsigned grid, M, bgrid;
	unsigned S;
	unsigned mach_cap, pool_cap;
	size_t units;
};
static unsigned mstreams_policy(size_t units, uint32_t last_bails, bool linear, unsigned pinned, unsigned light) {
	if(pinned) return pinned > H2G_MSTREAMS_MAX ? H2G_MSTREAMS_MAX : pinned;
	if(!linear || (size_t)last_bails * 1000 > units * 15) return H2G_MSTREAMS_MAX;
	return light < 1 ? 1u : light > H2G_MSTREAMS_MAX ? (unsigned)H2G_MSTREAMS_MAX : light;
}
extern "C" __attribute__((visibility("default"))) unsigned h2g_mstreams_policy(unsigned long long units, unsigned last_bails, int linear, unsigned pinned, unsigned light) {
	return mstreams_policy((size_t)units, last_bails, linear != 0, pinned, light);
}
static GoPlan go_plan(const h2g_stream* s, const h2g_align_params* p, bool paired) {
	GoPlan plan, *g = &plan;
	const size_t n_reads = s->cur().n_reads;
	g->linear = s->ix->dg.linear != 0;
	const bool ext_opts = pe_flags_from(*p) != H2G_PE_DEFAULT || p->min_frag_len != 0 || p->transcriptome_mapping_only || (p->avoid_pseudogene && !p->no_spliced_alignment);
	g->spl = !p->no_spliced_alignment || (p->use_haplotype && !g->linear) || ext_opts;
	const uint32_t maxsz = p->khits > p->kseeds ? p->khits : p->kseeds;
	g->L = &go_unit(g->linear, true, g->spl);
	const uint32_t* const caps = go_unit(g->linear, false, g->spl).caps, * const bcaps = g->L->caps;
	g->xl = p->khits > H2G_SELECT_CAP || maxsz > bcaps[0];
	g->big_main = maxsz > caps[0];
	g->U = &go_unit(g->linear, g->big_main, g->spl, g->xl);
	g->fast = s->tune.fast && !g->spl && !g->big_main && p->no_spliced_alignment && !p->secondary && !p->bowtie2_dp;
	g->fast_spl = s->tune.fast && s->tune.fast_spliced && g->linear && !p->no_spliced_alignment && !ext_opts && !g->big_main && !p->secondary && !p->bowtie2_dp;
	if(g->fast_spl) g->fast = true;
	g->second = !g->big_main && !s->tune.no_second_pass;
	size_t per_cu = (size_t)g->U->waves * 256 / g->U->threads;
	const size_t lds_blocks = (160u * 1024u) / (g->U->lds_ring_bytes + (paired ? 2u : 1u) * g->U->lds_pack_bytes);
	if(per_cu > lds_blocks) per_cu = lds_blocks;
	if(per_cu < 1) per_cu = 1;
	if(s->tune.blocks_per_cu > 0) per_cu = (size_t)s->tune.blocks_per_cu;
	const size_t want = (n_reads + g->U->slots - 1) / g->U->slots;
	size_t maxblocks = 256 * per_cu;
	if(g->big_main && maxblocks > 32) maxblocks = 32;
	if(g->xl && maxblocks > 12) maxblocks = 12;
	g->grid = (unsigned)(want < 1 ? 1 : (want > maxblocks ? maxblocks : want));
	g->M = s->mstreams ? s->mstreams : H2G_MSTREAMS_MAX;
	const bool mt_auto = s->tune.mach_total_auto != 0 && g->linear;
	g->units = paired ? n_reads : (n_reads + 1) / 2;
	const unsigned mach_total_now = mt_auto && (size_t)s->last_bails * 1000 > g->units * 15 ? 192u : s->tune.mach_total;
	g->S = mstreams_policy(g->units, s->last_bails, g->linear, s->mstreams, s->mstreams_light);
	g->mach_cap = mach_total_now / g->M;
	if(g->mach_cap > H2G_MACH_MAXGRID) g->mach_cap = H2G_MACH_MAXGRID;
	if(g->mach_cap < 1) g->mach_cap = 1;
	g->pool_cap = (mt_auto ? 192u : s->tune.mach_total) / g->M;
	if(g->pool_cap > H2G_MACH_MAXGRID) g->pool_cap = H2G_MACH_MAXGRID;
	if(g->pool_cap < g->mach_cap) g->pool_cap = g->mach_cap;
	g->bgrid = g->fast ? 2u : 4u;
	return plan;
}

struct FastPlan {
	bool use_am, mate_ho;
	bool ps0;
	const FastUnitDesc *FU, *DU;
	unsigned fgrid, mgrid, dgrid;
	uint32_t orphan_T;
	h2g_stream::FastPool* pool;
	size_t slot_bytes;
};
struct GoRun {
	GoArgs A; DExonTbl X; XlPairs XP;
	h2g_stream::RunSet* set;
	unsigned long long* cblk;
	unsigned lane;
	h2g_stream::MachStream* mach;
	hipStream_t ms;
	unsigned mach_grid;
	FastPlan f;
	uint32_t* ovl;
};

static void go_args(const h2g_stream* s, const h2g_align_params* p, bool paired, const GoPlan& g, GoRun* r) {
	const BatchCtx& b = s->cur();
	GoArgs& A = r->A;
	memset(&A, 0, sizeof A);
	A.g = dg_now(s->ix); A.ref = s->ix->dr; A.ls = dls_now(s->ix); A.alts = s->ix->dalts;
	if(p->max_alts_tried) A.alts.maxAltsTried = p->max_alts_tried;
	if(p->use_haplotype && !g.linear && A.alts.n) A.alts.has_splice |= 2u;
	A.rd1 = dreads(s); A.rd2 = A.rd1;
	if(paired) { A.rd2.codes = b.d_codes2; A.rd2.offs = b.d_offs2; A.rd2.quals = b.has_quals2 ? b.d_quals2 : nullptr; }
	if(b.has_seeds) { A.rd1.seeds = b.d_seeds; A.rd2.seeds = paired ? b.d_seeds + s->max_reads : b.d_seeds; }
	if(b.has_ids) { A.rd1.ids = b.d_ids; A.rd2.ids = b.d_ids; }
	if(b.has_qc) { A.rd1.qc = b.d_qc; A.rd2.qc = paired ? b.d_qc + s->max_reads : b.d_qc; }
	A.P = aln_params_from(*p, p->no_spliced_alignment != 0, g.linear);
	if(!p->no_spliced_alignment) { A.ssdb = s->ix->dssdb; A.rdid_base = p->first_read_id; }
	r->X = p->no_spliced_alignment ? DExonTbl() : s->ix->dexons;
	if(!p->no_spliced_alignment) { A.P.sc.donor_sum = s->ix->d_spl[0]; A.P.sc.acc_sum1 = s->ix->d_spl[1]; A.P.sc.acc_sum2 = s->ix->d_spl[2]; }
	A.names1 = b.d_names; A.noffs1 = b.d_name_offs; A.names2 = b.d_names2; A.noffs2 = b.d_name_offs2;
	A.paired = paired ? 1u : 0u;
}

static void go_select(h2g_stream* s, const GoPlan& g, GoRun* r) {
	r->set = &s->run[s->gen % (g.M + 1)];
	r->cblk = s->counters(*r->set);
	r->lane = g.fast ? s->gen % g.M : 0u;
	r->mach = &s->mach[r->lane % g.S];
}

static int go_rotation(h2g_stream* s, const GoPlan& g) {
	if(s->n_mst < g.S) s->n_mst = g.S;
	if(s->rot && s->rot != g.S && s->st2_busy) {
		for(unsigned j = 0; j < s->rot; j++) HIPCHK(hipEventRecord(s->mach[j].ev_rot, s->mst[j]));
		for(unsigned k = 0; k < g.S; k++) for(unsigned j = 0; j < s->rot; j++) if(j != k) HIPCHK(hipStreamWaitEvent(s->mst[k], s->mach[j].ev_rot, 0));
	}
	s->rot = g.S;
	return H2G_OK;
}

static int go_pools(h2g_stream* s, const h2g_align_params* p, const GoPlan& g, GoRun* r) {
	const size_t pgrid = g.fast && g.grid > g.pool_cap ? (size_t)g.pool_cap : (size_t)g.grid;
	int rc;
	if(g.fast && s->cur().n_reads >= 200000) {
		GoArgs scratch = r->A;
		for(unsigned k = 0; k < g.S && s->gen >= 1; k++) {
			h2g_stream::MachStream& m = s->mach[k];
			if((rc = go_pool_for(s, m.main, *g.U, pgrid * g.U->slots, pgrid * g.U->threads, p->bowtie2_dp, &scratch))) return rc;
			if(g.second && (rc = go_pool_for(s, m.second, *g.L, (size_t)g.bgrid * g.L->slots, (size_t)g.bgrid * g.L->threads, p->bowtie2_dp, &scratch))) return rc;
			if(!m.ovf_list) { HIPCHK(m.ovf_list.ensure(s->max_reads + 4)); HIPCHK(hipMemsetAsync(m.ovf_list + s->max_reads, 0, 16, s->stream_of(m))); }
		}
		for(unsigned k = 0; k < g.M + 1; k++) {
			h2g_stream::RunSet& b = s->run[k];
			HIPCHK(b.bail_list.ensure(s->max_reads + 4));
			HIPCHK(b.fast_args.ensure(1));
			HIPCHK(b.drain_args.ensure(1));
		}
	}
	return go_pool_for(s, r->mach->main, *g.U, pgrid * g.U->slots, pgrid * g.U->threads, p->bowtie2_dp, &r->A);
}

static int go_rows(h2g_stream* s, const h2g_align_params* p, bool paired, const GoPlan& g, GoRun* r) {
	BatchCtx& b = s->cur();
	GoArgs& A = r->A;
	memset(&A.O, 0, sizeof A.O);
	if(!paired) {
		HIPCHK(b.d_rout.ensure(s->max_reads));
		const uint32_t slots = p->khits;
		HIPCHK(b.d_aln.reserve(s->max_reads * (size_t)slots));
		b.aln_slots = slots;
		A.O.rout = b.d_rout; A.O.aln = b.d_aln; A.O.aln_slots = slots;
	} else {
		HIPCHK(b.d_pout.ensure(s->max_reads));
		uint32_t pslots = p->khits * 2 + 4;
		if(pslots < H2G_PAIR_RES_CAP) pslots = H2G_PAIR_RES_CAP;
		if(s->tune.pair_slots > 0) pslots = (uint32_t)s->tune.pair_slots;
		for(int m = 0; m < 2; m++) HIPCHK(b.d_paln[m].reserve(s->max_reads * (size_t)pslots));
		b.pair_slots = pslots;
		A.O.pout = b.d_pout; A.O.paln[0] = b.d_paln[0]; A.O.paln[1] = b.d_paln[1]; A.O.pair_slots = pslots;
		const size_t ovf_cap = s->max_reads / 4 > 65536 ? s->max_reads / 4 : 65536;
		if(!s->paln_ovf.fits(g.M, ovf_cap)) {
			HIPCHK(sync_mach(s));
			HIPCHK(hipStreamSynchronize(s->st));
			HIPCHK(s->paln_ovf.reset(g.M, ovf_cap));
		}
		A.O.ovf = s->paln_ovf;
	}
	memset(&r->XP, 0, sizeof r->XP);
	if(paired && g.xl) {
		const size_t xcap = s->max_reads * 64 > ((size_t)1 << 20) ? s->max_reads * 64 : ((size_t)1 << 20);
		if(s->d_xlp_at.size() < s->max_reads || !s->xlp.fits(g.M, xcap) || !s->d_xlp_cur) {
			HIPCHK(hipStreamSynchronize(s->st));
			HIPCHK(s->d_xlp_at.reset(s->max_reads));
			HIPCHK(s->xlp.reset(g.M, xcap));
			HIPCHK(s->d_xlp_cur.ensure(H2G_MSTREAMS_MAX));
		}
		HIPCHK(hipMemsetAsync(s->d_xlp_at, 0, b.n_reads * 4, s->st));
		HIPCHK(hipMemsetD32Async((hipDeviceptr_t)(s->d_xlp_cur + r->lane), (int)s->xlp.lo(r->lane), 1, s->st));
		r->XP.at = s->d_xlp_at; r->XP.list = s->xlp; r->XP.cursor = s->d_xlp_cur + r->lane; r->XP.cap = (uint32_t)s->xlp.hi(r->lane);
	}
	if(paired) s->xlp_pout = g.xl ? b.d_pout : (s->xlp_pout == b.d_pout ? nullptr : s->xlp_pout);
	return H2G_OK;
}

static int go_counters(h2g_stream* s, bool paired, const GoPlan& g, GoRun* r) {
	GoArgs& A = r->A;
	HIPCHK(hipStreamWaitEvent(s->st, r->set->ev_mach, 0));
	HIPCHK(hipMemsetAsync(r->cblk, 0, H2G_CNT_BLOCK * sizeof(unsigned long long), s->st));
	A.counters = r->cblk;
	A.work = reinterpret_cast<uint32_t*>(r->cblk + H2G_CNT_WORK_MAIN);
	if(paired) {
		A.O.ovf_cursor = reinterpret_cast<uint32_t*>(r->cblk + H2G_CNT_OVF_CURSOR);
		A.O.ovf_cap = (uint32_t)s->paln_ovf.hi(r->lane);
		if(r->lane) HIPCHK(hipMemsetD32Async((hipDeviceptr_t)A.O.ovf_cursor, (int)s->paln_ovf.lo(r->lane), 1, s->st));
	}
	A.list = nullptr; A.nlist = nullptr;
	if(s->tune.dbg_read >= 0) {
		HIPCHK(s->dbg_buf.ensure(1u << 20));
		HIPCHK(hipMemsetAsync(s->dbg_buf, 0, (1u << 20) * 4, s->st));
		A.dbg_buf = s->dbg_buf; A.dbg_read = (uint32_t)s->tune.dbg_read;
	}
	A.defer_overflow = g.second ? 1u : 0u;
	return H2G_OK;
}

static void fast_policy(h2g_stream* s, bool paired, const GoPlan& g, FastPlan* f) {
	const size_t n_reads = s->cur().n_reads;
	const bool linear = g.linear;
	*f = FastPlan();
	f->use_am = linear && paired && s->tune.align_mate != 0 && !g.fast_spl;
	f->FU = &fast_unit(linear, g.fast_spl, f->use_am);
	const unsigned NB = g.M + 1;
	for(unsigned back = 1; back < NB && back <= s->gen; back++) {
		const h2g_stream::RunSet& b = s->run[(s->gen - back) % NB];
		if(hipEventQuery(b.ev_bails) == hipSuccess) { s->last_bails = s->h_bail(b); break; }
	}
	(void)hipGetLastError();
	unsigned mach_div = s->tune.mach_div;
	if(mach_div == 0) {
		mach_div = 400;
		if(!linear) {
			const size_t units = paired ? n_reads : n_reads / 2;
			if(units >= 1000000) mach_div = 1600;
			else if(units > 500000) mach_div = 400 + (unsigned)((units - 500000) * 1200 / 500000);
		}
	}
	f->mgrid = (unsigned)((s->last_bails + mach_div - 1) / (mach_div ? mach_div : 1u));
	if(f->mgrid < s->tune.mach_min) f->mgrid = s->tune.mach_min;
	if(f->mgrid > g.mach_cap) f->mgrid = g.mach_cap;
	const size_t fwant = (n_reads + 127) / 128;
	unsigned reserve = s->tune.fast_reserve >= 0 ? (unsigned)s->tune.fast_reserve : g.S * f->mgrid;
	if(reserve > 192) reserve = 192;
	const unsigned fmax = 256 - reserve;
	f->fgrid = (unsigned)(fwant < 1 ? 1 : (fwant > fmax ? fmax : fwant));
	f->slot_bytes = (size_t)256 * f->FU->slots * f->FU->slot_bytes;
	f->orphan_T = s->tune.orphan >= 0 ? (uint32_t)s->tune.orphan : (g.units >= H2G_ORPHAN_MIN_UNITS ? (uint32_t)H2G_ORPHAN_T : 0u);
	if(f->orphan_T > f->FU->slots) f->orphan_T = f->FU->slots;
	if(f->FU->gws_bytes != 0) f->orphan_T = 0;
	f->dgrid = (unsigned)(s->tune.drain_grid < 1 ? 1 : s->tune.drain_grid);
	f->mate_ho = f->orphan_T != 0 && linear && paired && !f->use_am && !g.fast_spl && s->tune.mate_handover != 0;
	f->DU = &fast_unit(linear, g.fast_spl, f->use_am || f->mate_ho);
	f->pool = &s->fpool[f->orphan_T ? s->gen % H2G_FAST_POOLS : 0u];
	f->ps0 = linear && !g.fast_spl && (s->tune.ps0 < 0 ? H2G_DEFAULT_PS0 != 0 : s->tune.ps0 != 0);
}

static int fast_buffers(h2g_stream* s, const GoPlan& g, const FastPlan& f) {
	const size_t ocap = (size_t)256 * f.FU->slots, dbytes = (size_t)f.dgrid * f.DU->slots * f.DU->slot_bytes;
	const size_t dsc = g.linear ? 0 : (size_t)f.dgrid * f.FU->threads * (size_t)(2 * H2G_COMBINE_MAXLEN * sizeof(int64_t));
	h2g_stream::FastPool* const pools = f.orphan_T ? s->fpool : f.pool;
	const unsigned npools = f.orphan_T ? (unsigned)H2G_FAST_POOLS : 1u;
	bool need = f.pool->slots.size() < f.slot_bytes;
	if(f.orphan_T) {
		for(unsigned q = 0; q < npools; q++) need = need || pools[q].slots.size() < f.slot_bytes;
		need = need || s->d_drain_slots.size() < dbytes || s->d_drain_sc.size() < dsc;
		for(unsigned b = 0; b < g.M + 1; b++) need = need || !s->run[b].orphans || !s->run[b].drain_args;
		need = need || s->orphan_cap < ocap;
	}
	const size_t pswords = (size_t)s->max_reads * 4 * FG_PS0_WORDS;
	if(f.ps0) for(unsigned q = 0; q < npools; q++) need = need || pools[q].ps0.size() < pswords;
	if(!need) return H2G_OK;
	HIPCHK(hipStreamSynchronize(s->st)); HIPCHK(hipStreamSynchronize(s->dst)); for(unsigned k = 0; k < s->n_mst; k++) HIPCHK(hipStreamSynchronize(s->mst[k]));
	for(unsigned q = 0; q < npools; q++) {
		DevBuf<uint8_t>& fs = pools[q].slots;
		if(fs.size() < f.slot_bytes) { HIPCHK(fs.reserve(f.slot_bytes)); HIPCHK(hipMemsetAsync(fs, 0, f.slot_bytes, s->st)); }
		DevBuf<uint32_t>& ps = pools[q].ps0;
		if(f.ps0 && ps.size() < pswords) { HIPCHK(ps.reserve(pswords)); HIPCHK(hipMemsetAsync(ps, 0xff, pswords * 4, s->st)); }
	}
	if(f.orphan_T) {
		if(s->orphan_cap < ocap) { for(h2g_stream::RunSet& b : s->run) b.orphans = DevBuf<uint32_t>(); s->orphan_cap = ocap; }
		for(unsigned k = 0; k < g.M + 1; k++) {
			h2g_stream::RunSet& b = s->run[k];
			if(!b.orphans) { HIPCHK(b.orphans.ensure(s->orphan_cap + 4)); HIPCHK(hipMemsetAsync(b.orphans, 0, (s->orphan_cap + 4) * 4, s->st)); }
			HIPCHK(b.drain_args.ensure(1));
		}
		if(s->d_drain_slots.size() < dbytes) { HIPCHK(s->d_drain_slots.reserve(dbytes)); HIPCHK(hipMemsetAsync(s->d_drain_slots, 0, dbytes, s->st)); }
		if(s->d_drain_sc.size() < dsc) { HIPCHK(s->d_drain_sc.reserve(dsc)); HIPCHK(hipMemsetAsync(s->d_drain_sc, 0, dsc, s->st)); }
	}
	HIPCHK(hipStreamSynchronize(s->st));
	return H2G_OK;
}

static int fast_launch(h2g_stream* s, bool paired, const GoPlan& g, GoRun* r) {
	const FastPlan& f = r->f;
	const GoArgs& A = r->A;
	h2g_stream::RunSet& set = *r->set;
	HIPCHK(hipStreamWaitEvent(s->st, f.pool->ev_last, 0));
	HIPCHK(set.bail_list.ensure(s->max_reads + 4));
	uint32_t* const bl = set.bail_list;
	HIPCHK(hipMemsetAsync(bl + s->max_reads, 0, 16, s->st));
	FastArgs F;
	memset(&F, 0, sizeof F);
	F.g = A.g; F.ref = A.ref; F.ls = A.ls; F.rd1 = A.rd1; F.rd2 = A.rd2; F.P = A.P;
	F.names1 = A.names1; F.noffs1 = A.noffs1; F.names2 = A.names2; F.noffs2 = A.noffs2;
	F.slots = (uint32_t*)f.pool->slots.get();
	F.O.rout = A.O.rout; F.O.aln = A.O.aln; F.O.aln_slots = A.O.aln_slots; F.O.pout = A.O.pout; F.O.paln[0] = A.O.paln[0]; F.O.paln[1] = A.O.paln[1]; F.O.pair_slots = A.O.pair_slots;
	F.counters = r->cblk; F.work = reinterpret_cast<uint32_t*>(r->cblk + H2G_CNT_WORK_FAST);
	F.bail_list = bl; F.bail_count = bl + s->max_reads;
	F.total = (uint32_t)s->cur().n_reads; F.paired = paired ? 1u : 0u;
	F.alts = A.alts; F.gws_base = nullptr; F.gws_stride = 0; F.sc_base = nullptr;
	F.dbg_read = A.dbg_read; F.dbg_buf = A.dbg_buf;
	F.ps0 = f.ps0 ? f.pool->ps0.get() : nullptr;
	F.ssdb = A.ssdb; F.rdid_base = A.rdid_base;
	F.tail = g.linear && paired && s->tune.tail > 0 ? (uint32_t)s->tune.tail : 0u;
	if(!g.linear) {
		const size_t lanes = (size_t)256 * f.FU->threads;
		HIPCHK(s->d_fast_gws.reserve(lanes * f.FU->gws_bytes));
		HIPCHK(s->d_fast_sc.reserve(lanes * (size_t)(2 * H2G_COMBINE_MAXLEN * sizeof(int64_t))));
		F.gws_base = s->d_fast_gws; F.gws_stride = f.FU->gws_bytes; F.sc_base = s->d_fast_sc;
	}
	HIPCHK(set.fast_args.ensure(1));
	FastArgs D = F;
	if(f.orphan_T) {
		uint32_t* const ol = set.orphans;
		HIPCHK(hipMemsetAsync(ol + s->orphan_cap, 0, 16, s->st));
		F.orphan_T = f.orphan_T; F.orphan_list = ol; F.orphan_count = ol + s->orphan_cap; F.mate_handover = f.mate_ho ? 1u : 0u;
		D.adopt_slot_words = f.FU->slot_bytes / 4;
		if(s->tune.tail_auto) D.tail = g.linear && paired && (size_t)s->last_bails * 1000 > g.units * 15 ? (uint32_t)H2G_DEFAULT_TAIL : 0u;
		D.slots = (uint32_t*)s->d_drain_slots.get();
		D.adopt_list = ol; D.adopt_count = ol + s->orphan_cap; D.adopt_slots = F.slots;
		D.work = reinterpret_cast<uint32_t*>(r->cblk + H2G_CNT_WORK_DRAIN);
		D.cnt_off = H2G_CNT_DRAIN_OFF;
		D.total = 0;
		if(!g.linear) D.sc_base = s->d_drain_sc;
		s->orph_cur = ol + s->orphan_cap;
	}
	if(s->gen >= g.M + 1 && hipEventQuery(set.ev_fast) != hipSuccess) { (void)hipGetLastError(); HIPCHK(hipEventSynchronize(set.ev_fast)); }
	FastArgs* const hF = s->h_fast(set);
	*hF = F;
	HIPCHK(hipMemcpyAsync(set.fast_args, hF, sizeof F, hipMemcpyHostToDevice, s->st));
	if(f.orphan_T) {
		FastArgs* const hD = s->h_drain(set);
		*hD = D;
		HIPCHK(hipMemcpyAsync(set.drain_args, hD, sizeof D, hipMemcpyHostToDevice, s->st));
	}
	if(f.ps0 && h2g_ps0_launch(set.fast_args, F.total, paired, s->st) != 0) return set_err("go() first-search pre-pass launch", hipGetLastError());
	if(f.FU->launch(set.fast_args, f.fgrid, s->st) != 0) return set_err("go() fast pass launch", hipGetLastError());
	r->A.list = bl; r->A.nlist = bl + s->max_reads;
	return H2G_OK;
}

static int fast_handoff(h2g_stream* s, bool paired, const GoPlan& g, GoRun* r) {
	const FastPlan& f = r->f;
	h2g_stream::RunSet& set = *r->set;
	HIPCHK(hipEventRecord(set.ev_fast, s->st));
	r->ms = s->stream_of(*r->mach); s->st2_busy = true;
	if(f.mgrid < r->mach_grid) r->mach_grid = f.mgrid;
	if(f.orphan_T) {
		HIPCHK(hipStreamWaitEvent(s->dst, set.ev_fast, 0));
		HIPCHK(hipEventRecord(s->ev_dr[0], s->dst));
		if(f.DU->launch_drain(set.drain_args, f.dgrid, s->dst) != 0) return set_err("go() drain launch", hipGetLastError());
		HIPCHK(hipEventRecord(s->ev_dr[1], s->dst));
		HIPCHK(hipEventRecord(f.pool->ev_last, s->dst));
		HIPCHK(hipMemcpyAsync(&s->h_bail(set), set.bail_list + s->max_reads, 4, hipMemcpyDeviceToHost, s->dst));
		HIPCHK(hipEventRecord(set.ev_drain, s->dst));
		HIPCHK(hipEventRecord(set.ev_bails, s->dst));
		HIPCHK(hipStreamWaitEvent(r->ms, set.ev_drain, 0));
		s->ran_drain = true; s->dst_busy = true;
	} else {
		HIPCHK(hipMemcpyAsync(&s->h_bail(set), set.bail_list + s->max_reads, 4, hipMemcpyDeviceToHost, s->st));
		HIPCHK(hipEventRecord(set.ev_bails, s->st));
		HIPCHK(hipStreamWaitEvent(r->ms, set.ev_fast, 0));
	}
	return H2G_OK;
}

static int go_mach_lists(h2g_stream* s, const GoPlan& g, GoRun* r) {
	GoArgs& A = r->A;
	const unsigned lane = r->lane;
	s->ovf_cur = r->mach;
	HIPCHK(r->mach->ovf_list.ensure(s->max_reads + 4));
	r->ovl = r->mach->ovf_list;
	HIPCHK(hipMemsetAsync(r->ovl + s->max_reads, 0, 16, r->ms));
	const size_t lcap = s->max_reads > (1u << 20) ? s->max_reads : (size_t)(1u << 20);
	if(!s->ledits.fits(g.M, lcap) || !s->d_ledits_cur) {
		if(s->st2_busy) for(unsigned k = 0; k < s->n_mst; k++) HIPCHK(hipStreamSynchronize(s->mst[k]));
		HIPCHK(hipStreamSynchronize(s->st));
		HIPCHK(s->ledits.reset(g.M, lcap));
		HIPCHK(s->d_ledits_cur.ensure(H2G_MSTREAMS_MAX));
		for(unsigned m = 0; m < H2G_MSTREAMS_MAX; m++) HIPCHK(hipMemsetD32Async((hipDeviceptr_t)(s->d_ledits_cur + m), (int)(m < g.M ? s->ledits.lo(m) : 0), 1, s->st));
		HIPCHK(hipStreamSynchronize(s->st));
	}
	A.O.ledits = s->ledits; A.O.ledits_cursor = s->d_ledits_cur + lane; A.O.ledits_cap = (uint32_t)s->ledits.hi(lane);
	HIPCHK(hipMemsetD32Async((hipDeviceptr_t)A.O.ledits_cursor, (int)s->ledits.lo(lane), 1, r->ms));
	s->ledits_touched |= 1u << lane;
	if(g.second) { A.O.defer_list = r->ovl; A.O.defer_count = r->ovl + s->max_reads; }
	return H2G_OK;
}

static bool go_cold(const h2g_stream* s, const GoPlan& g, const GoRun& r) {
	for(unsigned k = 0; k < g.S; k++) if(&s->mach[k] != r.mach && !s->mach[k].warmed) return true;
	return false;
}
static int go_warmup(h2g_stream* s, const h2g_align_params* p, const GoPlan& g, const GoRun& r) {
	int rc;
	const size_t warm_rows = (size_t)1 << 16;
	if(!s->d_warm_cnt) { HIPCHK(s->d_warm_cnt.ensure(H2G_CNT_BLOCK)); HIPCHK(hipMemset(s->d_warm_cnt, 0, H2G_CNT_BLOCK * sizeof(unsigned long long))); }
	if(!s->d_warm_rows) { HIPCHK(s->d_warm_rows.ensure(warm_rows)); HIPCHK(hipMemset(s->d_warm_rows, 0, warm_rows)); }
	for(unsigned k = 0; k < g.S; k++) {
		h2g_stream::MachStream& m = s->mach[k];
		const hipStream_t ms = s->stream_of(m);
		if(&m == r.mach || m.warmed || !m.ovf_list) continue;
		GoArgs W1 = r.A;
		if((rc = go_pool_for(s, m.main, *g.U, (size_t)g.U->slots, (size_t)g.U->threads, p->bowtie2_dp, &W1))) return rc;
		W1.counters = s->d_warm_cnt; W1.work = reinterpret_cast<uint32_t*>(s->d_warm_cnt + H2G_CNT_WORK_MAIN);
		W1.list = reinterpret_cast<uint32_t*>(s->d_warm_rows.get()); W1.nlist = reinterpret_cast<uint32_t*>(s->d_warm_cnt + H2G_CNT_NO_SECOND);
		memset(&W1.O, 0, sizeof W1.O);
		W1.O.rout = reinterpret_cast<ReadOut*>(s->d_warm_rows.get()); W1.O.aln = reinterpret_cast<h2g_alnres*>(s->d_warm_rows.get()); W1.O.aln_slots = r.A.O.aln_slots;
		W1.O.pout = reinterpret_cast<PairOut*>(s->d_warm_rows.get()); W1.O.paln[0] = W1.O.paln[1] = reinterpret_cast<h2g_alnres*>(s->d_warm_rows.get()); W1.O.pair_slots = r.A.O.pair_slots;
		W1.O.ovf = reinterpret_cast<h2g_alnres*>(s->d_warm_rows.get()); W1.O.ledits = reinterpret_cast<h2g_edit*>(s->d_warm_rows.get());
		W1.O.ovf_cursor = reinterpret_cast<uint32_t*>(s->d_warm_cnt + H2G_CNT_OVF_CURSOR); W1.O.ledits_cursor = reinterpret_cast<uint32_t*>(s->d_warm_cnt + H2G_CNT_LEDITS_CURSOR);
		W1.defer_overflow = 0;
		HIPCHK(hipMemsetAsync(s->d_warm_cnt + H2G_CNT_NO_SECOND, 0, 8 * sizeof(unsigned long long), ms));
		if(g.U->launch(&W1, &r.X, nullptr, 1, ms) != 0) return set_err("go() warm-up launch", hipGetLastError());
		if(g.second) {
			GoArgs W2 = W1;
			if((rc = go_pool_for(s, m.second, *g.L, (size_t)g.L->slots, (size_t)g.L->threads, p->bowtie2_dp, &W2))) return rc;
			W2.work = reinterpret_cast<uint32_t*>(s->d_warm_cnt + H2G_CNT_WORK_SECOND);
			if(g.L->launch(&W2, &r.X, nullptr, 1, ms) != 0) return set_err("go() warm-up launch", hipGetLastError());
		}
		m.warmed = true;
	}
	s->st2_busy = true;
	return H2G_OK;
}

static int go_mach(h2g_stream* s, const h2g_align_params* p, const GoPlan& g, GoRun* r) {
	HIPCHK(hipEventRecord(s->tm[TM_MAIN0], r->ms));
	if(g.U->launch(&r->A, &r->X, &r->XP, r->mach_grid, r->ms) != 0) return set_err("go() launch", hipGetLastError());
	HIPCHK(hipEventRecord(s->tm[TM_MAIN1], r->ms));
	if(g.second) {
		GoArgs A2 = r->A;
		int rc;
		if((rc = go_pool_for(s, r->mach->second, *g.L, (size_t)g.bgrid * g.L->slots, (size_t)g.bgrid * g.L->threads, p->bowtie2_dp, &A2))) return rc;
		A2.counters = r->cblk + H2G_CNT_SECOND;
		A2.work = reinterpret_cast<uint32_t*>(r->cblk + H2G_CNT_WORK_SECOND);
		A2.list = r->ovl; A2.nlist = r->ovl + s->max_reads;
		A2.defer_overflow = 0; A2.O.defer_list = nullptr; A2.O.defer_count = nullptr;
		if(g.L->launch(&A2, &r->X, nullptr, g.bgrid, r->ms) != 0) return set_err("go() second pass launch", hipGetLastError());
	}
	HIPCHK(hipEventRecord(s->tm[TM_RUN1], r->ms));
	if(g.fast) { HIPCHK(hipEventRecord(r->set->ev_mach, r->ms)); r->mach->warmed = true; }
	return H2G_OK;
}

static h2g_status go_run(h2g_stream* s, const h2g_align_params* p, bool paired) {
	if(!s || !p) return H2G_ERR_ARG;
	int rc;
	if((rc = go_check(s, p, paired))) return rc;
	const GoPlan g = go_plan(s, p, paired);
	HIPCHK(hipSetDevice(s->ix->device));
	if(s->st2_busy && (s->last_paired != (paired ? 1 : 0) || memcmp(&s->last_p, p, sizeof *p) != 0)) HIPCHK(sync_mach(s));
	s->last_p = *p; s->last_paired = paired ? 1 : 0;
	GoRun r = {};
	go_args(s, p, paired, g, &r);
	go_select(s, g, &r);
	if(!g.fast) HIPCHK(sync_mach(s));
	else if((rc = go_rotation(s, g))) return rc;
	if((rc = go_pools(s, p, g, &r)) || (rc = go_rows(s, p, paired, g, &r))) return rc;
	(void)hipGetLastError();
	if((rc = go_counters(s, paired, g, &r))) return rc;
	HIPCHK(hipEventRecord(s->tm[TM_RUN0], s->st));
	s->ran_fast = g.fast;
	if(g.fast) {
		fast_policy(s, paired, g, &r.f);
		if((rc = fast_buffers(s, g, r.f)) || (rc = fast_launch(s, paired, g, &r))) return rc;
	}
	HIPCHK(hipEventRecord(s->tm[TM_FAST1], s->st));
	r.ms = s->st; r.mach_grid = g.grid;
	s->ran_drain = false;
	if(g.fast && (rc = fast_handoff(s, paired, g, &r))) return rc;
	if((rc = go_mach_lists(s, g, &r))) return rc;
	if(g.fast && s->cur().n_reads >= 200000 && s->gen >= 1 && go_cold(s, g, r) && (rc = go_warmup(s, p, g, r))) return rc;
	if((rc = go_mach(s, p, g, &r))) return rc;
	s->cnt_cur = r.cblk; s->gen++;
	HIPCHK(hipGetLastError());
	s->ran_align = true;
	return H2G_OK;
}

extern "C" h2g_status h2g_align_run(h2g_stream* s, const h2g_align_params* p) { return go_run(s, p, false); }
extern "C" h2g_status h2g_align_pairs_run(h2g_stream* s, const h2g_align_params* p) { return go_run(s, p, true); }

extern "C" h2g_status h2g_align_fetch(h2g_stream* s, h2g_read_result* res, h2g_alnres* aln, size_t first, size_t n) {
	if(s) HIPCHK(sync_mach(s));
	if(!s || !res || first + n > s->cur().n_reads || !s->cur().d_rout) return H2G_ERR_ARG;
	std::vector<ReadOut> tmp(n);
	HIPCHK(hipMemcpyAsync(tmp.data(), s->cur().d_rout + first, n * sizeof(ReadOut), hipMemcpyDeviceToHost, s->st));
	if(aln && n) {
		const uint32_t w = s->cur().aln_slots < H2G_ALN_CAP ? s->cur().aln_slots : H2G_ALN_CAP;
		HIPCHK(hipMemcpy2DAsync(aln, (size_t)H2G_ALN_CAP * sizeof(h2g_alnres), s->cur().d_aln + first * s->cur().aln_slots, (size_t)s->cur().aln_slots * sizeof(h2g_alnres),
		                        (size_t)w * sizeof(h2g_alnres), n, hipMemcpyDeviceToHost, s->st));
	}
	HIPCHK(sync_all(s));
	for(size_t i = 0; i < n; i++) {
		res[i].nres = tmp[i].nres; res[i].nselect = tmp[i].nselect; res[i].overflow = tmp[i].overflow;
		res[i].nrank = tmp[i].nrank; res[i].nsteps = tmp[i].nsteps; res[i].depth = tmp[i].depth;
		res[i].best = tmp[i].best; res[i].secbest = tmp[i].secbest; res[i].best_h2 = tmp[i].best_h2; res[i].secbest_h2 = tmp[i].secbest_h2;
	}
	return H2G_OK;
}

static h2g_status xlp_flag(h2g_stream* s, h2g_pair_result* res, size_t first, size_t n) {
	if(!s->xlp_pout || s->xlp_pout != s->cur().d_pout || n == 0) return H2G_OK;
	std::vector<uint32_t> at(n);
	HIPCHK(hipMemcpy(at.data(), s->d_xlp_at + first, n * 4, hipMemcpyDeviceToHost));
	for(size_t i = 0; i < n; i++) if(at[i]) res[i].overflow |= H2G_OVF_PAIR_LIST;
	return H2G_OK;
}
static h2g_status pairs_fetch_rows(h2g_stream* s, h2g_pair_result* res, h2g_alnres* aln1, h2g_alnres* aln2, size_t first, size_t n, bool callers_view) {
	if(s) HIPCHK(sync_mach(s));
	if(!s || !res || first + n > s->cur().n_reads || !s->cur().d_pout) return H2G_ERR_ARG;
	if((aln1 || aln2) && s->cur().pair_slots < H2G_PAIR_RES_CAP) return H2G_ERR_ARG;
	HIPCHK(hipMemcpyAsync(res, s->cur().d_pout + first, n * sizeof(PairOut), hipMemcpyDeviceToHost, s->st));
	for(int m = 0; m < 2 && n; m++) {
		h2g_alnres* dst = m == 0 ? aln1 : aln2;
		if(dst) HIPCHK(hipMemcpy2DAsync(dst, (size_t)H2G_PAIR_RES_CAP * sizeof(h2g_alnres), s->cur().d_paln[m] + first * s->cur().pair_slots, (size_t)s->cur().pair_slots * sizeof(h2g_alnres),
		                                (size_t)H2G_PAIR_RES_CAP * sizeof(h2g_alnres), n, hipMemcpyDeviceToHost, s->st));
	}
	HIPCHK(sync_all(s));
	if(callers_view) for(size_t i = 0; i < n; i++) if(res[i].pad) { res[i].overflow |= 4; res[i].pad = 0; }
	return xlp_flag(s, res, first, n);
}
extern "C" h2g_status h2g_align_pairs_fetch(h2g_stream* s, h2g_pair_result* res, h2g_alnres* aln1, h2g_alnres* aln2, size_t first, size_t n) { return pairs_fetch_rows(s, res, aln1, aln2, first, n, true); }

__global__ __launch_bounds__(256) void k_gather_aln(const h2g_alnres* src, uint32_t slots, const uint32_t* cnt, uint32_t cnt_stride,
                                                    const unsigned long long* offs, size_t n, h2g_alnres* dst,
                                                    const PairOut* pout = nullptr, const h2g_alnres* ovf = nullptr, int mate = 0)
{
	const size_t i = blockIdx.x * (size_t)blockDim.x + threadIdx.x;
	if(i >= n) return;
	uint32_t c = cnt[i * cnt_stride];
	const h2g_alnres* a = src + i * slots;
	if(pout && pout[i].pad) a = ovf + (pout[i].pad - 1u) + (mate ? pout[i].nres[0] : 0u);
	else if(c > slots) c = slots;
	h2g_alnres* d = dst + offs[i];
	for(uint32_t k = 0; k < c; k++) {
		d[k].fw = a[k].fw; d[k].tidx = a[k].tidx; d[k].toff = a[k].toff; d[k].len = a[k].len; d[k].trim5 = a[k].trim5; d[k].trim3 = a[k].trim3;
		d[k].nedits = a[k].nedits; d[k].splicescore = a[k].splicescore; d[k].score = a[k].score;
		for(uint32_t e = 0; e < a[k].nedits && e < H2G_MAX_EDITS; e++) d[k].edits[e] = a[k].edits[e];
	}
}
static uint64_t dense_offsets(const uint32_t* h_cnt, uint32_t h_stride, uint32_t slots, size_t n, uint64_t* offs, const uint32_t* h_pad = nullptr) {
	uint64_t tot = 0;
	for(size_t i = 0; i < n; i++) { offs[i] = tot; const uint32_t c = h_cnt[i * h_stride]; tot += (c < slots || (h_pad && h_pad[i * h_stride])) ? c : slots; }
	offs[n] = tot;
// ... 301 lines not shown
	}
	out->n_records = n;
	out->first_not_plain = UINT64_MAX;
	s->fq_stats.bytes_uploaded = n1 + n2;
	if(n == 0) { out->first_not_plain = 0; s->fq_stats.kernel_ms = ms_total; return H2G_OK; }
	struct Lay { size_t nlpos, lsz, nsz, src, bits, res; } lay[2];
	size_t at = 0;
	for(int m = 0; m < M; m++) {
		Lay& l = lay[m];
		l.nlpos = at; at = up16(at + (4 * n + 1) * 4);
		l.lsz = at;   at = up16(at + scan64_bytes(n + 1));
		l.nsz = at;   at = up16(at + scan64_bytes(n + 1));
		l.src = at;   at = up16(at + 3 * n * 4);
		l.bits = at;  at = up16(at + n);
		l.res = at;   at = up16(at + 16);
	}
	void* d_tab;
	if((rc = tmp_buf(s, 3, at, &d_tab))) return (h2g_status)rc;
	uint8_t* T = (uint8_t*)d_tab;
	const h2g_fq::Opts fo = {opts->trim5, opts->trim3, opts->phred64 ? 1u : 0u};
	static const uint32_t res0[4] = {0, 0xffffffffu, 0, 0};
	uint32_t hres[2][4];
	unsigned long long tot_l[2] = {0, 0}, tot_n[2] = {0, 0};
	uint32_t last_nl[2] = {0, 0};
	uint64_t known[2];
	HIPCHK(hipEventRecord(s->tm[TM_SET0], s->st));
	for(int m = 0; m < M; m++) {
		const Lay& l = lay[m];
		known[m] = std::min<uint64_t>(nl[m], 4 * n);
		HIPCHK(hipMemcpyAsync(T + l.res, res0, 16, hipMemcpyHostToDevice, s->st));
		const unsigned long long* v = (const unsigned long long*)((uint8_t*)d_cnt + cnt_at[m]);
		hipLaunchKernelGGL(k_fq_lines, dim3((unsigned)nblk[m]), dim3(256), 0, s->st, (const uint8_t*)d_text[m], (uint32_t)nt[m], v, (uint32_t*)(T + l.nlpos), known[m]);
		hipLaunchKernelGGL(k_fq_table, dim3((unsigned)((n + 1 + 255) / 256)), dim3(256), 0, s->st, (const char*)d_text[m], (uint32_t)nt[m], (const uint32_t*)(T + l.nlpos), known[m], (uint32_t)n, fo,
		                   (unsigned long long*)(T + l.lsz), (unsigned long long*)(T + l.nsz), (uint32_t*)(T + l.src), T + l.bits,
		                   m ? (const uint8_t*)(T + lay[0].bits) : (const uint8_t*)nullptr, (uint32_t*)(T + l.res));
		scan64(s, (unsigned long long*)(T + l.lsz), n + 1);
		scan64(s, (unsigned long long*)(T + l.nsz), n + 1);
	}
	HIPCHK(hipGetLastError());
	HIPCHK(hipEventRecord(s->tm[TM_SET1], s->st));
	for(int m = 0; m < M; m++) {
		const Lay& l = lay[m];
		HIPCHK(hipMemcpyAsync(hres[m], T + l.res, 16, hipMemcpyDeviceToHost, s->st));
		HIPCHK(hipMemcpyAsync(&tot_l[m], (unsigned long long*)(T + l.lsz) + n, 8, hipMemcpyDeviceToHost, s->st));
		HIPCHK(hipMemcpyAsync(&tot_n[m], (unsigned long long*)(T + l.nsz) + n, 8, hipMemcpyDeviceToHost, s->st));
		if(known[m] == 4 * n) HIPCHK(hipMemcpyAsync(&last_nl[m], (uint32_t*)(T + l.nlpos) + (4 * n - 1), 4, hipMemcpyDeviceToHost, s->st));
	}
	HIPCHK(sync_all(s));
	HIPCHK(hipEventElapsedTime(&ms, s->tm[TM_SET0], s->tm[TM_SET1])); ms_total += ms;
	s->fq_stats.kernel_ms = ms_total;
	const uint64_t consumed[2] = {known[0] == 4 * n ? (uint64_t)last_nl[0] + 1 : n1, M == 2 ? (known[1] == 4 * n ? (uint64_t)last_nl[1] + 1 : n2) : 0};
	out->consumed1 = consumed[0]; out->consumed2 = consumed[1];
	out->n_bases1 = tot_l[0]; out->n_bases2 = tot_l[1];
	out->n_name_bytes1 = tot_n[0]; out->n_name_bytes2 = tot_n[1];
	out->n_not_plain = (uint64_t)hres[0][0] + (M == 2 ? hres[1][0] : 0u);
	out->max_read_len = std::max(hres[0][2], M == 2 ? hres[1][2] : 0u);
	if(out->n_not_plain) { out->first_not_plain = std::min(hres[0][1], M == 2 ? hres[1][1] : 0xffffffffu); return H2G_OK; }
	out->first_not_plain = n;
	if(n > s->max_reads || tot_l[0] > s->max_bases || tot_l[1] > s->max_bases || tot_n[0] > 0xffffffffull || tot_n[1] > 0xffffffffull) {
		snprintf(g_err, sizeof g_err, "h2g_set_reads_fastq: %llu records of %llu / %llu bases exceed the stream's %zu reads / %zu bases, or their names 4 GB", (unsigned long long)n,
		         tot_l[0], tot_l[1], s->max_reads, s->max_bases);
		return H2G_ERR_ARG;
	}
	HIPCHK(B.reserve_names(tot_n[0], s->max_reads));
	if(M == 2) HIPCHK(B.ensure_mates(s->max_reads, s->max_bases, tot_n[1]));
	HIPCHK(hipEventRecord(s->tm[TM_SET0], s->st));
	for(int m = 0; m < M; m++) {
		const Lay& l = lay[m];
		const unsigned long long* lsz = (const unsigned long long*)(T + l.lsz);
		const unsigned long long* nsz = (const unsigned long long*)(T + l.nsz);
		const uint32_t* src = (const uint32_t*)(T + l.src);
		uint8_t* codes = m ? B.d_codes2 : B.d_codes;
		uint8_t* quals = (uint8_t*)(m ? B.d_quals2 : B.d_quals).get();
		uint8_t* names = (uint8_t*)(m ? B.d_names2 : B.d_names).get();
		hipLaunchKernelGGL(k_fq_offs, dim3((unsigned)((n + 1 + 255) / 256)), dim3(256), 0, s->st, lsz, nsz, (uint32_t)n, m ? B.d_offs2 : B.d_offs, m ? B.d_name_offs2 : B.d_name_offs);
		if(tot_l[m]) hipLaunchKernelGGL(k_fq_write<true>, dim3(grid_for((tot_l[m] + 15) / 16, 256)), dim3(256), 0, s->st, (const uint8_t*)d_text[m], lsz, src + n, src + 2 * n, (uint32_t)n, (uint64_t)tot_l[m],
		                                fo.phred64, codes, quals);
		if(tot_n[m]) hipLaunchKernelGGL(k_fq_write<false>, dim3(grid_for((tot_n[m] + 15) / 16, 256)), dim3(256), 0, s->st, (const uint8_t*)d_text[m], nsz, src, (const uint32_t*)nullptr, (uint32_t)n,
		                                (uint64_t)tot_n[m], 0u, names, (uint8_t*)nullptr);
		s->fq_stats.bytes_written += 2 * tot_l[m] + tot_n[m] + 2 * (n + 1) * 4;
	}
	HIPCHK(hipGetLastError());
	HIPCHK(hipEventRecord(s->tm[TM_SET1], s->st));
	HIPCHK(sync_all(s));
	HIPCHK(hipEventElapsedTime(&ms, s->tm[TM_SET0], s->tm[TM_SET1])); ms_total += ms;
	s->fq_stats.kernel_ms = ms_total;
	B.n_reads = n;
	B.max_read_len = out->max_read_len;
	B.has_quals = true;
	B.has_names = true;
	B.has_mates = M == 2;
	B.has_quals2 = M == 2;
	return H2G_OK;
}
extern "C" h2g_status h2g_get_fastq_stats(h2g_stream* s, h2g_fastq_stats* out) {
	if(!s || !out) return H2G_ERR_ARG;
	*out = s->fq_stats;
	return H2G_OK;
}

extern "C" h2g_status h2g_fetch_read_set(h2g_stream* s, int mate, size_t* n_reads, size_t* n_bases, size_t* n_name_bytes, uint8_t* codes, uint32_t* offs, char* quals, char* names,
                                         uint32_t* name_offs)
{
	if(!s || mate < 0 || mate > 1) return H2G_ERR_ARG;
	HIPCHK(sync_all(s));
	const BatchCtx& B = s->cur();
	const size_t n = B.n_reads;
	if(n_reads) *n_reads = n;
	if(n_bases) *n_bases = 0;
	if(n_name_bytes) *n_name_bytes = 0;
	if(n == 0) return H2G_OK;
	if(mate == 1 && !B.has_mates) return H2G_ERR_ARG;
	const uint8_t* dc = mate ? B.d_codes2 : B.d_codes;
	const uint32_t* dof = mate ? B.d_offs2 : B.d_offs;
	const char* dq = mate ? B.d_quals2 : B.d_quals;
	const char* dn = mate ? B.d_names2 : B.d_names;
	const uint32_t* dno = mate ? B.d_name_offs2 : B.d_name_offs;
	const bool hq = mate ? B.has_quals2 : B.has_quals, hn = mate ? true : B.has_names;
	uint32_t nb = 0, nn = 0;
	HIPCHK(hipSetDevice(s->ix->device));
	HIPCHK(hipMemcpyAsync(&nb, dof + n, 4, hipMemcpyDeviceToHost, s->st));
	if(hn) HIPCHK(hipMemcpyAsync(&nn, dno + n, 4, hipMemcpyDeviceToHost, s->st));
	HIPCHK(hipStreamSynchronize(s->st));
	if(n_bases) *n_bases = nb;
	if(n_name_bytes) *n_name_bytes = nn;
	if((quals && !hq) || ((names || name_offs) && !hn)) return H2G_ERR_ARG;
	if(codes && nb) HIPCHK(hipMemcpyAsync(codes, dc, nb, hipMemcpyDeviceToHost, s->st));
	if(offs) HIPCHK(hipMemcpyAsync(offs, dof, (n + 1) * 4, hipMemcpyDeviceToHost, s->st));
	if(quals && nb) HIPCHK(hipMemcpyAsync(quals, dq, nb, hipMemcpyDeviceToHost, s->st));
	if(names && nn) HIPCHK(hipMemcpyAsync(names, dn, nn, hipMemcpyDeviceToHost, s->st));
	if(name_offs) HIPCHK(hipMemcpyAsync(name_offs, dno, (n + 1) * 4, hipMemcpyDeviceToHost, s->st));
	HIPCHK(hipStreamSynchronize(s->st));
	return H2G_OK;
}

extern "C" h2g_status h2g_align_pairs_fetch_compact(h2g_stream* s, h2g_pair_result* res, uint8_t* rec1, size_t cap1, uint64_t* boffs1, uint8_t* rec2, size_t cap2, uint64_t* boffs2,
                                                    size_t first, size_t n)
{
	if(s) HIPCHK(sync_mach(s));
	if(!s || !res || !rec1 || !rec2 || !boffs1 || !boffs2 || first + n > s->cur().n_reads || !s->cur().d_pout) return H2G_ERR_ARG;
	if(n == 0) { boffs1[0] = boffs2[0] = 0; return H2G_OK; }
	HIPCHK(hipSetDevice(s->ix->device));
	static_assert(offsetof(PairOut, nres) == 0 && sizeof(h2g_pair_result) == sizeof(PairOut), "PairOut layout");
	const uint32_t* cnt = reinterpret_cast<const uint32_t*>(s->cur().d_pout + first);
	const uint32_t* xat = s->xlp_pout && s->xlp_pout == s->cur().d_pout ? s->d_xlp_at + first : nullptr;
	void *d_o1 = nullptr, *d_o2 = nullptr, *d_b1 = nullptr, *d_b2 = nullptr;
	int rc;
	if((rc = compact_offsets(s, s->cur().d_paln[0] + first * s->cur().pair_slots, s->cur().pair_slots, cnt, sizeof(PairOut) / 4, n, 0, s->cur().d_pout + first, 0, &d_o1, xat)) ||
	   (rc = compact_offsets(s, s->cur().d_paln[1] + first * s->cur().pair_slots, s->cur().pair_slots, cnt + 1, sizeof(PairOut) / 4, n, 2, s->cur().d_pout + first, 1, &d_o2))) return (h2g_status)rc;
	HIPCHK(hipMemcpyAsync(boffs1, d_o1, (n + 1) * 8, hipMemcpyDeviceToHost, s->st));
	HIPCHK(hipMemcpyAsync(boffs2, d_o2, (n + 1) * 8, hipMemcpyDeviceToHost, s->st));
	HIPCHK(hipMemcpyAsync(res, s->cur().d_pout + first, n * sizeof(PairOut), hipMemcpyDeviceToHost, s->st));
	HIPCHK(hipStreamSynchronize(s->st));
	for(size_t i = 0; i < n; i++) if(res[i].pad) { res[i].overflow &= ~4u; res[i].pad = 0; }
	if(boffs1[n] > cap1 || boffs2[n] > cap2) return H2G_ERR_ARG;
	if((rc = tmp_buf(s, 1, boffs1[n] + 8, &d_b1)) || (rc = tmp_buf(s, 3, boffs2[n] + 8, &d_b2))) return (h2g_status)rc;
	const unsigned g = (unsigned)((n + 255) / 256);
	if(boffs1[n]) hipLaunchKernelGGL(k_compact_gather, dim3(g), dim3(256), 0, s->st, s->cur().d_paln[0] + first * s->cur().pair_slots, s->cur().pair_slots, cnt, (uint32_t)(sizeof(PairOut) / 4),
	                                 (const unsigned long long*)d_o1, n, (uint8_t*)d_b1, s->cur().d_pout + first, (const h2g_alnres*)s->paln_ovf, 0,
	                                 xat, xat ? (const uint32_t*)s->xlp : (const uint32_t*)nullptr);
	if(boffs2[n]) hipLaunchKernelGGL(k_compact_gather, dim3(g), dim3(256), 0, s->st, s->cur().d_paln[1] + first * s->cur().pair_slots, s->cur().pair_slots, cnt + 1, (uint32_t)(sizeof(PairOut) / 4),
	                                 (const unsigned long long*)d_o2, n, (uint8_t*)d_b2, s->cur().d_pout + first, (const h2g_alnres*)s->paln_ovf, 1);
	HIPCHK(hipGetLastError());
	if(boffs1[n]) HIPCHK(hipMemcpyAsync(rec1, d_b1, boffs1[n], hipMemcpyDeviceToHost, s->st));
	if(boffs2[n]) HIPCHK(hipMemcpyAsync(rec2, d_b2, boffs2[n], hipMemcpyDeviceToHost, s->st));
	HIPCHK(hipStreamSynchronize(s->st));
// ... 298 lines not shown
		uploaded += he.size() * sizeof(SamHardEntry) + hl.size() * sizeof(h2g_sam_line) + n_aux;
		HIPCHK(hipMemsetAsync(d_bad, 0, 8, s->st));
		HIPCHK(hipMemsetAsync(s->d_sam[0], 0, n_lines * sizeof(h2g_sam_line), s->st));
		HIPCHK(hipEventRecord(s->ev_plan[2], s->st));
		if(!he.empty()) hipLaunchKernelGGL(k_sam_plan_scatter, dim3((unsigned)((he.size() + 255) / 256)), dim3(256), 0, s->st, (const SamHardEntry*)s->d_plan[3].get(), he.size(), n, (const uint8_t*)d_cls, v, d_hsrc);
		hipLaunchKernelGGL(k_scan_tiles, dim3((unsigned)ntiles_r), dim3(256), 0, s->st, v, n + 1, ts);
		hipLaunchKernelGGL(k_scan_tile_sums, dim3(1), dim3(1024), 0, s->st, ts, ntiles_r);
		hipLaunchKernelGGL(k_scan_add, dim3(g1), dim3(256), 0, s->st, v, n + 1, (const unsigned long long*)ts);
		hipLaunchKernelGGL(k_sam_plan_place, dim3((unsigned)((n + 255) / 256)), dim3(256), 0, s->st, (const uint8_t*)d_cls, (const unsigned long long*)v, (const uint32_t*)d_hsrc,
		                   (const h2g_sam_line*)s->d_plan[0].get(), (const h2g_sam_line*)s->d_plan[4].get(), hl.size(), n, n_lines, (h2g_sam_line*)s->d_sam[0].get(), d_ends, d_bad);
		HIPCHK(hipGetLastError());
		HIPCHK(hipEventRecord(s->ev_plan[3], s->st));
		hr = sam_text_tail(s, paired, n_lines, n_aux, short_lines ? nullptr : out, short_lines ? 0 : cap, used, short_lines ? nullptr : line_offs, uploaded, true);
		if(hr != H2G_OK) return hr;
		if(short_lines) return H2G_ERR_ARG;
		if(*used && (!out || *used > cap)) return H2G_ERR_ARG;
	}
	if(line_ends) {
		if(n_lines) { HIPCHK(hipMemcpyAsync(line_ends, d_ends, n * 8, hipMemcpyDeviceToHost, s->st)); HIPCHK(hipStreamSynchronize(s->st)); }
		else memset(line_ends, 0, n * 8);
	}
	guard.p = nullptr;
	h2g_plan::plan_commit(S, part, cls.data(), n);
	float ka = 0, kb = 0;
	if(hipEventElapsedTime(&ka, s->ev_plan[0], s->ev_plan[1]) != hipSuccess) ka = 0;
	if(n_lines == 0 || hipEventElapsedTime(&kb, s->ev_plan[2], s->ev_plan[3]) != hipSuccess) kb = 0;
	(void)hipGetLastError();
	s->plan_stats.device_planned = n - hard.size(); s->plan_stats.host_planned = hard.size(); s->plan_stats.n_lines = n_lines; s->plan_stats.bytes_uploaded = uploaded;
	for(const h2g_sam_line& d : hl) s->plan_stats.whole_lines += (d.bits & H2G_SAM_LINE_WHOLE_LINE) != 0;
	s->plan_stats.plan_kernel_ms = ka + kb; s->plan_stats.host_plan_ms = host_ms;
	s->plan_classes.swap(cls);
	return H2G_OK;
}
extern "C" h2g_status h2g_sam_text_unpaired_planned(h2g_stream* s, const h2g_sam* S, const uint8_t* codes, const uint32_t* offs, const char* quals, const char* nb, const uint32_t* noffs, size_t n,
                                                    const h2g_read_result* res, const uint8_t* rec, const uint64_t* boffs, char* out, size_t cap, size_t* used, uint64_t* line_offs, size_t line_cap,
                                                    size_t* n_lines, uint64_t* line_ends)
{
	const h2g_plan::HostSets rd = {{codes, nullptr}, {offs, nullptr}, {quals, nullptr}, {nb, nullptr}, {noffs, nullptr}};
	return sam_text_planned(s, S, false, rd, n, res, rec, boffs, nullptr, nullptr, 0, out, cap, used, line_offs, line_cap, n_lines, line_ends);
}
extern "C" h2g_status h2g_sam_text_paired_planned(h2g_stream* s, const h2g_sam* S, const uint8_t* codes1, const uint32_t* offs1, const char* quals1, const char* nb1, const uint32_t* noffs1,
                                                  const uint8_t* codes2, const uint32_t* offs2, const char* quals2, const char* nb2, const uint32_t* noffs2, size_t n, const h2g_pair_result* res,
                                                  const uint8_t* rec1, const uint64_t* boffs1, const uint8_t* rec2, const uint64_t* boffs2, uint32_t khits,
                                                  char* out, size_t cap, size_t* used, uint64_t* line_offs, size_t line_cap, size_t* n_lines, uint64_t* line_ends)
{
	const h2g_plan::HostSets rd = {{codes1, codes2}, {offs1, offs2}, {quals1, quals2}, {nb1, nb2}, {noffs1, noffs2}};
	return sam_text_planned(s, S, true, rd, n, res, rec1, boffs1, rec2, boffs2, khits, out, cap, used, line_offs, line_cap, n_lines, line_ends);
}
extern "C" h2g_status h2g_get_sam_plan_stats(h2g_stream* s, h2g_sam_plan_stats* out, uint8_t* classes, size_t cap) {
	if(!s || !out) return H2G_ERR_ARG;
	*out = s->plan_stats;
	if(classes) {
		if(cap < s->plan_classes.size()) return H2G_ERR_ARG;
		if(!s->plan_classes.empty()) memcpy(classes, s->plan_classes.data(), s->plan_classes.size());
	}
	return H2G_OK;
}

extern "C" void* h2g_host_alloc(size_t bytes) { void* p = nullptr; if(hipHostMalloc(&p, bytes ? bytes : 1, hipHostMallocPortable) != hipSuccess) { (void)hipGetLastError(); return nullptr; } return p; }
extern "C" void h2g_host_free(void* p) { if(p) (void)hipHostFree(p); }

extern "C" h2g_status h2g_align_fetch_long_edits(h2g_stream* s, h2g_edit* out, size_t cap, size_t* n) {
	if(!s || !n) return H2G_ERR_ARG;
	*n = 0;
	if(!s->ran_align || !s->ledits || !s->d_ledits_cur) return H2G_OK;
	HIPCHK(hipSetDevice(s->ix->device));
	HIPCHK(sync_mach(s));
	HIPCHK(hipStreamSynchronize(s->st));
	uint32_t cur[H2G_MSTREAMS_MAX];
	HIPCHK(hipMemcpy(cur, s->d_ledits_cur, sizeof cur, hipMemcpyDeviceToHost));
	PartSpan span[H2G_MSTREAMS_MAX];
	const size_t hi = part_spans(cur, s->ledits_touched, s->ledits.parts, s->ledits.cap, span);
	*n = hi;
	if(hi == 0) return H2G_OK;
	if(!out || cap < hi) return H2G_ERR_ARG;
	for(unsigned m = 0; m < s->ledits.parts; m++)
		if(span[m].end > span[m].lo) HIPCHK(hipMemcpy(out + span[m].lo, s->ledits + span[m].lo, (span[m].end - span[m].lo) * sizeof(h2g_edit), hipMemcpyDeviceToHost));
	return H2G_OK;
}

extern "C" __attribute__((visibility("default"))) int h2g_stream_tune(h2g_stream* s, const char* key, long v) {
	if(!s || !key) return H2G_ERR_ARG;
	HIPCHK(sync_all(s));
	for(unsigned k_ = 0; k_ < s->n_mst; k_++) HIPCHK(hipStreamSynchronize(s->mst[k_]));
	const std::string k(key);
	if(k == "mstreams") { s->mstreams = clamp_mstreams(v); s->gen = 0; return H2G_OK; }
	if(k == "mstreams_light") { s->mstreams_light = clamp_mstreams(v); return H2G_OK; }
	if(k == "mach_total" && v <= 0) { s->tune.mach_total_auto = 1; s->tune.mach_total = H2G_MACH_TOTAL; return H2G_OK; }
	if(k == "drain_grid") v = v < 1 ? 1 : v > 128 ? 128 : v;
	for(const Knob& kn : g_knobs) if(k == kn.key) {
		kn.set(s->tune, v);
		if(kn.is_auto) s->tune.*kn.is_auto = 0;
		return H2G_OK;
	}
	return H2G_ERR_ARG;
}

extern "C" __attribute__((visibility("default"))) long h2g_stream_probe(const h2g_stream* s, const char* key) {
	if(!s || !key) return -1;
	const std::string k(key);
	if(k == "mstreams_rotation") return (long)s->rot;
	if(k == "mstreams_used") return (long)s->n_mst;
	if(k == "mstreams_created") { long n = 0; for(hipStream_t m : s->mst) n += m != nullptr; return n; }
	if(k == "lanes") return (long)(s->mstreams ? s->mstreams : H2G_MSTREAMS_MAX);
	if(k == "pools") { long n = 0; for(const h2g_stream::MachStream& m : s->mach) n += bool(m.main.ws) + bool(m.second.ws); return n; }
	return -1;
}

extern "C" __attribute__((visibility("default"))) int h2g_go_debug_trace(h2g_stream* s, uint32_t* out, uint32_t cap_words) {
	if(s) HIPCHK(sync_mach(s));
	if(!s || !out || !s->dbg_buf) return H2G_ERR_ARG;
	HIPCHK(sync_all(s));
	HIPCHK(hipMemcpy(out, s->dbg_buf, (size_t)cap_words * 4, hipMemcpyDeviceToHost));
	return H2G_OK;
}

extern "C" __attribute__((visibility("default"))) int h2g_go_prof(h2g_stream* s, unsigned long long* out48) {
	if(!s || !out48) return H2G_ERR_ARG;
	HIPCHK(sync_all(s));
	HIPCHK(hipMemcpy(out48, s->cnt_cur + H2G_CNT_PROF_GO, 80 * sizeof(unsigned long long), hipMemcpyDeviceToHost));
	return H2G_OK;
}

extern "C" __attribute__((visibility("default"))) int h2g_go_fast_prof(h2g_stream* s, unsigned long long* out72 ) {
	if(!s || !out72) return H2G_ERR_ARG;
	HIPCHK(sync_all(s));
	HIPCHK(hipMemcpy(out72, s->cnt_cur + H2G_CNT_PROF_FAST, 48 * sizeof(unsigned long long), hipMemcpyDeviceToHost));
	HIPCHK(hipMemcpy(out72 + 48, s->cnt_cur + H2G_CNT_FAST_BAIL_WHY, 24 * sizeof(unsigned long long), hipMemcpyDeviceToHost));
	HIPCHK(hipMemcpy(out72 + 72, s->cnt_cur + H2G_CNT_PROF_FAST_SITE, 64 * sizeof(unsigned long long), hipMemcpyDeviceToHost));
	return H2G_OK;
}
#ifdef H2G_GO_PROF
extern "C" __attribute__((visibility("default"))) int h2g_go_fast_prof_bins(h2g_stream* s, unsigned long long* out256) {
	if(!s || !out256) return H2G_ERR_ARG;
	HIPCHK(sync_all(s));
	HIPCHK(hipMemcpy(out256, s->cnt_cur + H2G_CNT_PROF_FAST_BINS, 256 * sizeof(unsigned long long), hipMemcpyDeviceToHost));
	return H2G_OK;
}
#endif

extern "C" h2g_status h2g_get_counters(h2g_stream* s, h2g_counters* c) {
	if(!s || !c) return H2G_ERR_ARG;
	HIPCHK(sync_all(s));
	unsigned long long v[16];
	unsigned long long* const cb = s->ran_align ? s->cnt_cur : s->d_counters;
	HIPCHK(hipMemcpy(v, cb, 8 * sizeof(unsigned long long), hipMemcpyDeviceToHost));
	HIPCHK(hipMemcpy(v + 8, cb + (s->ran_align ? H2G_CNT_SECOND : H2G_CNT_NO_SECOND), 8 * sizeof(unsigned long long), hipMemcpyDeviceToHost));
	s->last.n_rank = v[0] + v[8]; s->last.n_side = v[1] + v[9]; s->last.n_sa_steps = v[2] + v[10]; s->last.n_ext = v[3];
	s->last.n_aligned = v[4] + v[12];
	uint32_t nsecond = 0;
	if(s->ovf_cur->ovf_list && s->ran_align) HIPCHK(hipMemcpy(&nsecond, s->ovf_cur->ovf_list + s->max_reads, 4, hipMemcpyDeviceToHost));
	s->last.n_second_pass = nsecond;
	s->last.n_overflow = nsecond ? v[13] : v[5];
	s->last.n_queries = s->cur().n_reads * 2;
	float t = 0;
	if(s->ran_seed) {
		if(hipEventElapsedTime(&t, s->tm[TM_SEED0], s->tm[TM_SEED_MID]) == hipSuccess) s->last.ms_search = t;
		if(hipEventElapsedTime(&t, s->tm[TM_SEED_MID], s->tm[TM_SEED1]) == hipSuccess) s->last.ms_resolve_extend = t;
	}
	if(s->ran_align && hipEventElapsedTime(&t, s->tm[TM_MAIN0], s->tm[TM_MAIN1]) == hipSuccess) s->last.ms_align_kernel = t;
	if(s->ran_align && hipEventElapsedTime(&t, s->tm[TM_RUN0], s->tm[TM_RUN1]) == hipSuccess) s->last.ms_align = t;
	s->last.n_fast = 0; s->last.n_fast_bail = 0; s->last.ms_fast_kernel = 0; s->last.pad_ = 0; s->last.n_fast_side = 0; s->last.n_fast_sa_steps = 0;
	s->last.ms_drain_kernel = 0; s->last.pad2_ = 0; s->last.n_drain_side = 0; s->last.n_drain_sa_steps = 0; s->last.n_adopted = 0;
	if(s->ran_align && s->ran_fast) {
		unsigned long long f[2], fc[4];
		HIPCHK(hipMemcpy(f, s->cnt_cur + H2G_CNT_FAST_DONE, sizeof f, hipMemcpyDeviceToHost));
		HIPCHK(hipMemcpy(fc, s->cnt_cur + H2G_CNT_FAST_RANK, sizeof fc, hipMemcpyDeviceToHost));
		s->last_bails = (uint32_t)f[1];
		s->last.n_fast = f[0]; s->last.n_fast_bail = f[1];
		s->last.n_fast_side = fc[1]; s->last.n_fast_sa_steps = fc[2];
		s->last.n_rank += fc[0]; s->last.n_side += fc[1]; s->last.n_sa_steps += fc[2]; s->last.n_aligned += fc[3];
		if(hipEventElapsedTime(&t, s->tm[TM_RUN0], s->tm[TM_FAST1]) == hipSuccess) s->last.ms_fast_kernel = t;
		if(s->ran_drain) {
			unsigned long long dc[4]; uint32_t nad = 0;
			HIPCHK(hipMemcpy(dc, s->cnt_cur + H2G_CNT_FAST_RANK + H2G_CNT_DRAIN_OFF, sizeof dc, hipMemcpyDeviceToHost));
			HIPCHK(hipMemcpy(&nad, s->orph_cur, 4, hipMemcpyDeviceToHost));
			s->last.n_drain_side = dc[1]; s->last.n_drain_sa_steps = dc[2]; s->last.n_adopted = nad;
			s->last.n_rank += dc[0]; s->last.n_side += dc[1]; s->last.n_sa_steps += dc[2]; s->last.n_aligned += dc[3];
			if(hipEventElapsedTime(&t, s->ev_dr[0], s->ev_dr[1]) == hipSuccess) s->last.ms_drain_kernel = t;
		}
	}
	(void)hipGetLastError();
	*c = s->last;
	return H2G_OK;
}
```

Before: 226.2 million.

## Allow ps0 pre-pass on a side stream and pass args by value

Adds an option to launch the first-search pre-pass kernel on a separate machine stream, ordered by a reads-written event and the pool's last-use event and joined back into the main stream before the fast pass. The kernel now takes a compact by-value argument struct instead of reading FastArgs through a device pointer, and uses a grid-stride loop over tiles so the grid size can be tuned. Both the side-stream option and the grid knob default to off, so the default path keeps the same stream and grid and only changes how arguments are passed. The side-stream path needs extra event bookkeeping and a count of held streams so later synchronisation also covers the side stream.

```diff
diff --git a/hisat2_amd/api.py b/hisat2_amd/api.py
--- a/hisat2_amd/api.py
+++ b/hisat2_amd/api.py
@@ -522,6 +522,13 @@
     return int(f(int(units), int(last_bails), int(bool(linear)), int(pinned), int(light)))
 
 
+def ps0_side_policy(linear, spliced, ps0, S, knob=-1):
+    f = lib().h2g_ps0_side_policy
+    f.argtypes = [C.c_int, C.c_int, C.c_int, C.c_uint, C.c_int]
+    f.restype = C.c_uint
+    return int(f(int(bool(linear)), int(bool(spliced)), int(bool(ps0)), int(S), int(knob)))
+
+
 class WindowPlan:
     def __init__(self, length, step, first_rdid=0):
         self.h = C.c_void_p()
diff --git a/hisat2_amd/csrc/h2g_go_args.h b/hisat2_amd/csrc/h2g_go_args.h
--- a/hisat2_amd/csrc/h2g_go_args.h
+++ b/hisat2_amd/csrc/h2g_go_args.h
@@ -176,7 +176,14 @@
 	uint32_t rdid_base;
 	uint32_t* ps0;
 };
-extern "C" int h2g_ps0_launch(const FastArgs* a, uint32_t units, bool paired, hipStream_t st);
+struct Ps0Args {
+	h2g::DGfm g;
+	h2g::DReads rd1, rd2;
+	uint32_t pseudogeneStop, anchorStop, khits, paired;
+	uint32_t* ps0;
+	uint32_t units;
+};
+extern "C" int h2g_ps0_launch(const Ps0Args* a, unsigned grid, hipStream_t st);
 struct FastUnitDesc {
 	int (*launch)(const FastArgs* a, unsigned grid, hipStream_t);
 	int (*launch_drain)(const FastArgs* a, unsigned grid, hipStream_t);
diff --git a/hisat2_amd/csrc/h2g_k_ps0.hip b/hisat2_amd/csrc/h2g_k_ps0.hip
--- a/hisat2_amd/csrc/h2g_k_ps0.hip
+++ b/hisat2_amd/csrc/h2g_k_ps0.hip
@@ -4,45 +4,51 @@
 
 #define PS0_THREADS 256
 
-__global__ __launch_bounds__(PS0_THREADS, 6) void k_ps0(const FastArgs* __restrict__ A, uint32_t units)
+__global__ __launch_bounds__(PS0_THREADS, 6) void k_ps0(const Ps0Args A)
 {
 	__shared__ uint32_t s_pk[H2G_PK_WORDS * PS0_THREADS];
-	const bool paired = A->paired != 0;
+	const bool paired = A.paired != 0;
 	const uint32_t sh = paired ? 2u : 1u;
-	const uint32_t t = blockIdx.x * PS0_THREADS + threadIdx.x;
-	const uint32_t unit = t >> sh, x = t & ((1u << sh) - 1u), mate = x >> 1;
+	const uint32_t tiles = (uint32_t)((((unsigned long long)A.units << sh) + PS0_THREADS - 1) / PS0_THREADS);
 	const uint32_t lane = threadIdx.x & 63u;
-	const bool live = unit < units;
-	const DReads& rd = mate ? A->rd2 : A->rd1;
 	uint32_t* const pk = s_pk + (threadIdx.x & ~1u);
-	bool ok = true;
-	uint32_t rl = 0;
-	if(live) {
-		rl = rd.offs[unit + 1] - rd.offs[unit];
-		if((x & 1u) == 0) {
-			ok = fg_pack_read(rd, unit, pk, PS0_THREADS);
-			if(rd.qc && !rd.qc[unit]) ok = false;
+	for(uint32_t tile = blockIdx.x; tile < tiles; tile += gridDim.x) {
+		const uint32_t t = tile * PS0_THREADS + threadIdx.x;
+		const uint32_t unit = t >> sh, x = t & ((1u << sh) - 1u), mate = x >> 1;
+		const bool live = unit < A.units;
+		const DReads& rd = mate ? A.rd2 : A.rd1;
+		bool ok = true;
+		uint32_t rl = 0;
+		if(live) {
+			rl = rd.offs[unit + 1] - rd.offs[unit];
+			if((x & 1u) == 0) {
+				ok = fg_pack_read(rd, unit, pk, PS0_THREADS);
+				if(rd.qc && !rd.qc[unit]) ok = false;
+			}
 		}
+		__syncthreads();
+		const unsigned long long bad = __ballot(!ok);
+		const bool absent = ((bad >> (lane & ~((1u << sh) - 1u))) & ((1ull << (1u << sh)) - 1ull)) != 0;
+		if(live) {
+			uint32_t rec[FG_PS0_WORDS] = {FG_PS0_ABSENT, FG_PS0_ABSENT, FG_PS0_ABSENT, FG_PS0_ABSENT};
+			if(!absent) {
+				SeqView sv;
+				sv.fwc = nullptr; sv.q = nullptr; sv.len = rl; sv.fw = (x & 1u) == 0;
+				sv.pk = pk; sv.pk_stride = PS0_THREADS; sv.pk_nomask = true;
+				h2g_fm_hit fh;
+				partial_search_item(A.g, sv, 0, A.pseudogeneStop != 0, A.anchorStop != 0, A.khits, &fh);
+				fg_ps0_pack(fh, rec);
+			}
+			*reinterpret_cast<uint4*>(A.ps0 + ((size_t)unit * 4 + x) * FG_PS0_WORDS) = make_uint4(rec[0], rec[1], rec[2], rec[3]);
+		}
+		__syncthreads();
 	}
-	__syncthreads();
-	const unsigned long long bad = __ballot(!ok);
-	const bool absent = ((bad >> (lane & ~((1u << sh) - 1u))) & ((1ull << (1u << sh)) - 1ull)) != 0;
-	if(!live) return;
-	uint32_t rec[FG_PS0_WORDS] = {FG_PS0_ABSENT, FG_PS0_ABSENT, FG_PS0_ABSENT, FG_PS0_ABSENT};
-	if(!absent) {
-		SeqView sv;
-		sv.fwc = nullptr; sv.q = nullptr; sv.len = rl; sv.fw = (x & 1u) == 0;
-		sv.pk = pk; sv.pk_stride = PS0_THREADS; sv.pk_nomask = true;
-		h2g_fm_hit fh;
-		partial_search_item(A->g, sv, 0, A->P.pseudogeneStop != 0, A->P.anchorStop != 0, A->P.khits, &fh);
-		fg_ps0_pack(fh, rec);
-	}
-	*reinterpret_cast<uint4*>(A->ps0 + ((size_t)unit * 4 + x) * FG_PS0_WORDS) = make_uint4(rec[0], rec[1], rec[2], rec[3]);
 }
 
-extern "C" int h2g_ps0_launch(const FastArgs* a, uint32_t units, bool paired, hipStream_t st) {
-	if(units == 0) return 0;
-	const unsigned long long lanes = (unsigned long long)units * (paired ? 4u : 2u);
-	hipLaunchKernelGGL(k_ps0, dim3((unsigned)((lanes + PS0_THREADS - 1) / PS0_THREADS)), dim3(PS0_THREADS), 0, st, a, units);
+extern "C" int h2g_ps0_launch(const Ps0Args* a, unsigned grid, hipStream_t st) {
+	if(a->units == 0) return 0;
+	const unsigned long long lanes = (unsigned long long)a->units * (a->paired ? 4u : 2u);
+	if(grid == 0) grid = (unsigned)((lanes + PS0_THREADS - 1) / PS0_THREADS);
+	hipLaunchKernelGGL(k_ps0, dim3(grid), dim3(PS0_THREADS), 0, st, *a);
 	return (int)hipGetLastError();
 }
diff --git a/hisat2_amd/csrc/h2g_kernels.hip b/hisat2_amd/csrc/h2g_kernels.hip
--- a/hisat2_amd/csrc/h2g_kernels.hip
+++ b/hisat2_amd/csrc/h2g_kernels.hip
@@ -108,6 +108,10 @@
 #ifndef H2G_DEFAULT_PS0
 #define H2G_DEFAULT_PS0 1
 #endif
+#ifndef H2G_PS0_SIDE_DEFAULT
+#define H2G_PS0_SIDE_DEFAULT 0
+#endif
+#define H2G_PS0_GRID_DEFAULT 0
 #define H2G_DEFAULT_ALIGN_MATE 0
 #define H2G_DEFAULT_FAST_SPLICED 0
 #define H2G_MACH_MAXGRID 48u
@@ -123,6 +127,7 @@
 	DevBuf<uint32_t> d_seeds; bool has_seeds = false, has_seeds2 = false;
 	DevBuf<uint8_t> d_qc; bool has_qc = false;
 	DevBuf<uint32_t> d_ids; bool has_ids = false;
+	DevEvent ev_reads;
 	hipError_t ensure_reads(size_t max_reads, size_t max_bases) {
 		hipError_t e = d_codes.ensure(max_bases + 64);
 		if(e == hipSuccess) e = d_quals.ensure(max_bases + 64);
@@ -165,6 +170,7 @@
 		DevEvent ev_fast, ev_mach;
 		DevEvent ev_bails;
 		DevEvent ev_drain;
+		DevEvent ev_ps0;
 		DevBuf<uint32_t> bail_list;
 		DevBuf<uint32_t> orphans;
 		DevBuf<FastArgs> fast_args, drain_args;
@@ -209,13 +215,16 @@
 	DevBuf<uint8_t> d_drain_sc;
 	bool dst_busy = false;
 	DevEvent ev_dr[2];
+	DevEvent ev_ps[2];
+	unsigned ps_side = 0;
+	unsigned n_held = 0;
 	bool ran_drain = false;
 	const uint32_t* orph_cur = nullptr;
 	DevBuf<uint8_t> d_fast_gws;
 	DevBuf<uint8_t> d_fast_sc;
 	bool ran_fast = false;
 	struct Tune { int fast, blocks_per_cu, pair_slots, no_second_pass; unsigned mach_div, mach_min, mach_total; int mach_total_auto = 1; int fast_reserve; long dbg_read;
-	              int tail, tail_auto = 1, align_mate, orphan, drain_grid, mate_handover, ps0, fast_spliced; } tune = {};
+	              int tail, tail_auto = 1, align_mate, orphan, drain_grid, mate_handover, ps0, ps0_side, ps0_grid, fast_spliced; } tune = {};
 	h2g_align_params last_p; int last_paired = -1;
 	DevBuf<uint8_t> d_sw_ws;
 	DevBuf<SwLaneState> d_sw_states;
@@ -246,7 +255,7 @@
 	~h2g_stream() {
 		if(st) (void)hipStreamSynchronize(st);
 		if(dst) (void)hipStreamSynchronize(dst);
-		for(unsigned k = 0; k < n_mst; k++) (void)hipStreamSynchronize(mst[k]);
+		for(unsigned k = 0; k < n_held; k++) (void)hipStreamSynchronize(mst[k]);
 	}
 };
 struct StreamFree { void operator()(h2g_stream* s) const { h2g_stream_free(s); } };
@@ -819,6 +828,8 @@
 	H2G_KNOB("drain_grid",     "H2G_DRAIN_GRID",         H2G_DRAIN_GRID,           drain_grid,     nullptr),
 	H2G_KNOB("mate_handover",  "H2G_FAST_MATE_HANDOVER", -1,                       mate_handover,  nullptr),
 	H2G_KNOB("ps0",            "H2G_FAST_PS0",           -1,                       ps0,            nullptr),
+	H2G_KNOB("ps0_side",       "H2G_FAST_PS0_SIDE",      -1,                       ps0_side,       nullptr),
+	H2G_KNOB("ps0_grid",       "H2G_PS0_GRID",           H2G_PS0_GRID_DEFAULT,     ps0_grid,       nullptr),
 	H2G_KNOB("fast_spliced",   "H2G_FAST_SPLICED",       H2G_DEFAULT_FAST_SPLICED, fast_spliced,   nullptr),
 	H2G_KNOB("mach_total",     "H2G_MACH_TOTAL",         H2G_MACH_TOTAL,           mach_total,     &h2g_stream::Tune::mach_total_auto),
 	H2G_KNOB("fast_reserve",   "H2G_FAST_RESERVE",       H2G_FAST_RESERVE_DEFAULT, fast_reserve,   nullptr),
@@ -839,8 +850,10 @@
 	HIPCHK(s->h_fast_args.ensure(2 * H2G_NBUF));
 	HIPCHK(s->h_bails.ensure(H2G_NBUF)); for(int k = 0; k < H2G_NBUF; k++) s->h_bails[k] = 0;
 	for(h2g_stream::RunSet& b : s->run) { HIPCHK(b.ev_fast.create(hipEventDisableTiming)); HIPCHK(b.ev_mach.create(hipEventDisableTiming)); HIPCHK(b.ev_bails.create(hipEventDisableTiming)); HIPCHK(b.ev_drain.create(hipEventDisableTiming)); }
+	for(h2g_stream::RunSet& b : s->run) HIPCHK(b.ev_ps0.create(hipEventDisableTiming));
+	for(BatchCtx& b : s->batch) HIPCHK(b.ev_reads.create(hipEventDisableTiming));
 	for(h2g_stream::FastPool& fp : s->fpool) HIPCHK(fp.ev_last.create(hipEventDisableTiming));
-	for(int k = 0; k < 2; k++) HIPCHK(s->ev_dr[k].create());
+	for(int k = 0; k < 2; k++) { HIPCHK(s->ev_dr[k].create()); HIPCHK(s->ev_ps[k].create()); }
 	for(DevEvent& e : s->tm) HIPCHK(e.create());
 	HIPCHK(s->d_counters.ensure(H2G_NBUF * H2G_CNT_BLOCK));
 	HIPCHK(hipMemset(s->d_counters, 0, s->d_counters.bytes()));
@@ -866,7 +879,7 @@
 
 static hipError_t sync_mach(h2g_stream* s) {
 	if(!s->st2_busy) return hipSuccess;
-	for(unsigned k = 0; k < s->n_mst; k++) { const hipError_t e = hipStreamSynchronize(s->mst[k]); if(e != hipSuccess) return e; }
+	for(unsigned k = 0; k < s->n_held; k++) { const hipError_t e = hipStreamSynchronize(s->mst[k]); if(e != hipSuccess) return e; }
 	s->st2_busy = false;
 	return hipSuccess;
 }
@@ -915,6 +928,8 @@
 	*out = s->d_tmp[slot];
 	return e == hipSuccess ? H2G_OK : set_err("tmp_buf", e);
 }
+
+static hipError_t reads_written(h2g_stream* s, BatchCtx& B) { return hipEventRecord(B.ev_reads, s->st); }
 
 extern "C" h2g_status h2g_set_reads(h2g_stream* s, const uint8_t* codes, const uint32_t* offs, const char* quals, size_t n) {
 	if(s) HIPCHK(sync_all(s));
@@ -930,6 +945,7 @@
 	HIPCHK(hipMemcpyAsync(B.d_offs, offs, (n + 1) * 4, hipMemcpyHostToDevice, s->st));
 	B.has_quals = quals != nullptr;
 	if(quals) HIPCHK(hipMemcpyAsync(B.d_quals, quals, nb, hipMemcpyHostToDevice, s->st));
+	HIPCHK(reads_written(s, B));
 	HIPCHK(sync_all(s));
 	B.n_reads = n;
 	B.has_names = false;
@@ -2049,6 +2065,7 @@
 	if(quals2) HIPCHK(hipMemcpyAsync(B.d_quals2, quals2, offs2[n], hipMemcpyHostToDevice, s->st));
 	HIPCHK(hipMemcpyAsync(B.d_names2, nb2, noffs2[n], hipMemcpyHostToDevice, s->st));
 	HIPCHK(hipMemcpyAsync(B.d_name_offs2, noffs2, (n + 1) * 4, hipMemcpyHostToDevice, s->st));
+	HIPCHK(reads_written(s, B));
 	HIPCHK(sync_all(s));
 	B.has_mates = true;
 	return H2G_OK;
@@ -2158,6 +2175,7 @@
 	k_win_meta<<<grid_for(n + 1, 256), 256, 0, s->st>>>((const h2g_win::DSeg*)d_segs, (uint32_t)n_segs, len, step, (uint32_t)n, (const char*)d_pre, B.d_offs, B.d_ids, B.d_name_offs, B.d_names);
 	HIPCHK(hipGetLastError());
 	HIPCHK(hipEventRecord(s->tm[TM_SET1], s->st));
+	HIPCHK(reads_written(s, B));
 	HIPCHK(sync_all(s));
 	s->win_stats.bytes_uploaded = (hi - lo) + ds.size() * sizeof(h2g_win::DSeg) + n_prefix_bytes;
 	s->win_stats.bytes_written = n_bytes + (n + 1) * 8 + n * 4 + nb;
@@ -2215,6 +2233,7 @@
 	HIPCHK(B.d_qc.ensure(2 * s->max_reads));
 	if(pass1) HIPCHK(hipMemcpyAsync(B.d_qc, pass1, n, hipMemcpyHostToDevice, s->st)); else HIPCHK(hipMemsetAsync(B.d_qc, 1, n, s->st));
 	if(pass2) HIPCHK(hipMemcpyAsync(B.d_qc + s->max_reads, pass2, n, hipMemcpyHostToDevice, s->st)); else HIPCHK(hipMemsetAsync(B.d_qc + s->max_reads, 1, n, s->st));
+	HIPCHK(reads_written(s, B));
 	HIPCHK(sync_all(s));
 	B.has_qc = true;
 	return H2G_OK;
@@ -2351,6 +2370,14 @@
 }
 extern "C" __attribute__((visibility("default"))) unsigned h2g_mstreams_policy(unsigned long long units, unsigned last_bails, int linear, unsigned pinned, unsigned light) {
 	return mstreams_policy((size_t)units, last_bails, linear != 0, pinned, light);
+}
+static unsigned ps0_side_policy(bool linear, bool spliced, bool ps0, unsigned S, int knob) {
+	const int j = knob < 0 ? H2G_PS0_SIDE_DEFAULT : knob;
+	if(!linear || spliced || !ps0 || j < 1 || j >= H2G_MSTREAMS_MAX || (unsigned)j < S) return 0;
+	return (unsigned)j;
+}
+extern "C" __attribute__((visibility("default"))) unsigned h2g_ps0_side_policy(int linear, int spliced, int ps0, unsigned S, int knob) {
+	return ps0_side_policy(linear != 0, spliced != 0, ps0 != 0, S, knob);
 }
 static GoPlan go_plan(const h2g_stream* s, const h2g_align_params* p, bool paired) {
 	GoPlan plan, *g = &plan;
@@ -2396,6 +2423,7 @@
 struct FastPlan {
 	bool use_am, mate_ho;
 	bool ps0;
+	unsigned ps_side;
 	const FastUnitDesc *FU, *DU;
 	unsigned fgrid, mgrid, dgrid;
 	uint32_t orphan_T;
@@ -2443,6 +2471,7 @@
 
 static int go_rotation(h2g_stream* s, const GoPlan& g) {
 	if(s->n_mst < g.S) s->n_mst = g.S;
+	if(s->n_held < s->n_mst) s->n_held = s->n_mst;
 	if(s->rot && s->rot != g.S && s->st2_busy) {
 		for(unsigned j = 0; j < s->rot; j++) HIPCHK(hipEventRecord(s->mach[j].ev_rot, s->mst[j]));
 		for(unsigned k = 0; k < g.S; k++) for(unsigned j = 0; j < s->rot; j++) if(j != k) HIPCHK(hipStreamWaitEvent(s->mst[k], s->mach[j].ev_rot, 0));
@@ -2574,6 +2603,7 @@
 	f->DU = &fast_unit(linear, g.fast_spl, f->use_am || f->mate_ho);
 	f->pool = &s->fpool[f->orphan_T ? s->gen % H2G_FAST_POOLS : 0u];
 	f->ps0 = linear && !g.fast_spl && (s->tune.ps0 < 0 ? H2G_DEFAULT_PS0 != 0 : s->tune.ps0 != 0);
+	f->ps_side = ps0_side_policy(linear, g.fast_spl, f->ps0, g.S, s->tune.ps0_side);
 }
 
 static int fast_buffers(h2g_stream* s, const GoPlan& g, const FastPlan& f) {
@@ -2591,7 +2621,7 @@
 	const size_t pswords = (size_t)s->max_reads * 4 * FG_PS0_WORDS;
 	if(f.ps0) for(unsigned q = 0; q < npools; q++) need = need || pools[q].ps0.size() < pswords;
 	if(!need) return H2G_OK;
-	HIPCHK(hipStreamSynchronize(s->st)); HIPCHK(hipStreamSynchronize(s->dst)); for(unsigned k = 0; k < s->n_mst; k++) HIPCHK(hipStreamSynchronize(s->mst[k]));
+	HIPCHK(hipStreamSynchronize(s->st)); HIPCHK(hipStreamSynchronize(s->dst)); for(unsigned k = 0; k < s->n_held; k++) HIPCHK(hipStreamSynchronize(s->mst[k]));
 	for(unsigned q = 0; q < npools; q++) {
 		DevBuf<uint8_t>& fs = pools[q].slots;
 		if(fs.size() < f.slot_bytes) { HIPCHK(fs.reserve(f.slot_bytes)); HIPCHK(hipMemsetAsync(fs, 0, f.slot_bytes, s->st)); }
@@ -2665,7 +2695,28 @@
 		*hD = D;
 		HIPCHK(hipMemcpyAsync(set.drain_args, hD, sizeof D, hipMemcpyHostToDevice, s->st));
 	}
-	if(f.ps0 && h2g_ps0_launch(set.fast_args, F.total, paired, s->st) != 0) return set_err("go() first-search pre-pass launch", hipGetLastError());
+	if(f.ps0) {
+		Ps0Args PA;
+		memset(&PA, 0, sizeof PA);
+		PA.g = F.g; PA.rd1 = F.rd1; PA.rd2 = F.rd2;
+		PA.pseudogeneStop = F.P.pseudogeneStop; PA.anchorStop = F.P.anchorStop; PA.khits = F.P.khits; PA.paired = F.paired;
+		PA.ps0 = F.ps0; PA.units = F.total;
+		const unsigned pgrid = s->tune.ps0_grid > 0 ? (unsigned)s->tune.ps0_grid : 0u;
+		const hipStream_t ps = f.ps_side ? s->mst[f.ps_side].get() : s->st.get();
+		if(f.ps_side) {
+			if(s->n_held <= f.ps_side) s->n_held = f.ps_side + 1;
+			HIPCHK(hipStreamWaitEvent(ps, s->cur().ev_reads, 0));
+			HIPCHK(hipStreamWaitEvent(ps, f.pool->ev_last, 0));
+			HIPCHK(hipEventRecord(s->ev_ps[0], ps));
+		}
+		if(h2g_ps0_launch(&PA, pgrid, ps) != 0) return set_err("go() first-search pre-pass launch", hipGetLastError());
+		if(f.ps_side) {
+			HIPCHK(hipEventRecord(s->ev_ps[1], ps));
+			HIPCHK(hipEventRecord(set.ev_ps0, ps));
+			HIPCHK(hipStreamWaitEvent(s->st, set.ev_ps0, 0));
+			s->ps_side = f.ps_side;
+		}
+	}
 	if(f.FU->launch(set.fast_args, f.fgrid, s->st) != 0) return set_err("go() fast pass launch", hipGetLastError());
 	r->A.list = bl; r->A.nlist = bl + s->max_reads;
 	return H2G_OK;
@@ -2689,6 +2740,7 @@
 		HIPCHK(hipStreamWaitEvent(r->ms, set.ev_drain, 0));
 		s->ran_drain = true; s->dst_busy = true;
 	} else {
+		HIPCHK(hipEventRecord(f.pool->ev_last, s->st));
 		HIPCHK(hipMemcpyAsync(&s->h_bail(set), set.bail_list + s->max_reads, 4, hipMemcpyDeviceToHost, s->st));
 		HIPCHK(hipEventRecord(set.ev_bails, s->st));
 		HIPCHK(hipStreamWaitEvent(r->ms, set.ev_fast, 0));
@@ -2792,7 +2844,7 @@
 	(void)hipGetLastError();
 	if((rc = go_counters(s, paired, g, &r))) return rc;
 	HIPCHK(hipEventRecord(s->tm[TM_RUN0], s->st));
-	s->ran_fast = g.fast;
+	s->ran_fast = g.fast; s->ps_side = 0;
 	if(g.fast) {
 		fast_policy(s, paired, g, &r.f);
 		if((rc = fast_buffers(s, g, r.f)) || (rc = fast_launch(s, paired, g, &r))) return rc;
@@ -3260,6 +3312,7 @@
 	}
 	HIPCHK(hipGetLastError());
 	HIPCHK(hipEventRecord(s->tm[TM_SET1], s->st));
+	HIPCHK(reads_written(s, B));
 	HIPCHK(sync_all(s));
 	HIPCHK(hipEventElapsedTime(&ms, s->tm[TM_SET0], s->tm[TM_SET1])); ms_total += ms;
 	s->fq_stats.kernel_ms = ms_total;
@@ -3724,7 +3777,7 @@
 extern "C" __attribute__((visibility("default"))) int h2g_stream_tune(h2g_stream* s, const char* key, long v) {
 	if(!s || !key) return H2G_ERR_ARG;
 	HIPCHK(sync_all(s));
-	for(unsigned k_ = 0; k_ < s->n_mst; k_++) HIPCHK(hipStreamSynchronize(s->mst[k_]));
+	for(unsigned k_ = 0; k_ < s->n_held; k_++) HIPCHK(hipStreamSynchronize(s->mst[k_]));
 	const std::string k(key);
 	if(k == "mstreams") { s->mstreams = clamp_mstreams(v); s->gen = 0; return H2G_OK; }
 	if(k == "mstreams_light") { s->mstreams_light = clamp_mstreams(v); return H2G_OK; }
@@ -3743,6 +3796,7 @@
 	const std::string k(key);
 	if(k == "mstreams_rotation") return (long)s->rot;
 	if(k == "mstreams_used") return (long)s->n_mst;
+	if(k == "ps0_side") return (long)s->ps_side;
 	if(k == "mstreams_created") { long n = 0; for(hipStream_t m : s->mst) n += m != nullptr; return n; }
 	if(k == "lanes") return (long)(s->mstreams ? s->mstreams : H2G_MSTREAMS_MAX);
 	if(k == "pools") { long n = 0; for(const h2g_stream::MachStream& m : s->mach) n += bool(m.main.ws) + bool(m.second.ws); return n; }
@@ -3813,6 +3867,7 @@
 		s->last.n_fast_side = fc[1]; s->last.n_fast_sa_steps = fc[2];
 		s->last.n_rank += fc[0]; s->last.n_side += fc[1]; s->last.n_sa_steps += fc[2]; s->last.n_aligned += fc[3];
 		if(hipEventElapsedTime(&t, s->tm[TM_RUN0], s->tm[TM_FAST1]) == hipSuccess) s->last.ms_fast_kernel = t;
+		if(s->ps_side && hipEventElapsedTime(&t, s->ev_ps[0], s->ev_ps[1]) == hipSuccess) s->last.ms_fast_kernel += t;
 		if(s->ran_drain) {
 			unsigned long long dc[4]; uint32_t nad = 0;
 			HIPCHK(hipMemcpy(dc, s->cnt_cur + H2G_CNT_FAST_RANK + H2G_CNT_DRAIN_OFF, sizeof dc, hipMemcpyDeviceToHost));
```

Result: slower. 216.7 million (-4.2%).
